# ChuhanZhou/News_Recommendation_Model

Measured on AMD Instinct MI355X. Metric: train impressions/sec, higher is better.
Workload: dtype f32

## Files before the change

### include/nrm_hotpath.h

```cpp
#ifndef NRM_HOTPATH_H
#define NRM_HOTPATH_H

#ifdef __cplusplus
extern "C" {
#endif

#define NRM_ABI_VERSION 7
#define NRM_OK 0
#define NRM_EINVAL (-1)
#define NRM_ELAUNCH (-2)

typedef void* nrm_stream_t;

int nrm_abi_version(void);
const char* nrm_last_error(void);
int nrm_build_flags(void);
const char* nrm_source_digest(void);
const char* nrm_build_info(void);


#define NRM_MMA_F32 0
#define NRM_MMA_BF16 1
#define NRM_MMA_BF16X3 2
long nrm_pwattn_packed_floats(int D);
int nrm_pwattn_pack_wp(const float* fc1_weight, int ld, int D, int mma, float* packed, nrm_stream_t stream);
int nrm_pwattn_fwd(const float* t, const float* h, const float* u, const float* v, const float* packed_wp,
                   const float* w2, const float* b2, float* z, float* s,
                   int B, int T, int H, int D, int mma, nrm_stream_t stream);

#define NRM_DZ_F32 0
#define NRM_DZ_HL4 1
int nrm_pwattn_bwd_dz(float* z_inout, const float* ds, const float* w2, float* dw2, float* db2, float* du, float* dv,
                      int B, int T, int H, int D, int dz_format, nrm_stream_t stream);
int nrm_pwattn_bwd_nsplit(int B, int T, int H, int D, int mma);
int nrm_pwattn_bwd_contract(const float* dz, const float* t, const float* h, const float* wp, int ldwp,
                            float* dt, float* dh, float* ws,
                            int B, int T, int H, int D, int passes, int mma, int dz_format, nrm_stream_t stream);
int nrm_pwattn_bwd_form(int T, int H, int D, int pass, int mma, int dz_format);
int nrm_pwattn_bwd_rw_supported(int D, int mma);
long nrm_pwattn_bwd_rw_packed_floats(int D, int mma);
int nrm_pwattn_bwd_rw_pack(const float* fc1_weight, int ld, int D, int mma, float* packed, nrm_stream_t stream);
int nrm_pwattn_bwd_rw_dtdh(const float* dz_hl4, const float* t, const float* h, const float* packed, float* dt, float* dh,
                           int B, int T, int H, int D, int mma, nrm_stream_t stream);

int nrm_pwattn_bwd_dp_supported(int D, int H);
long nrm_pwattn_bwd_dp_packed_floats(int D, int H);
int nrm_pwattn_bwd_dp_pack(const float* fc1_weight, int ld, int D, int H, float* packed, nrm_stream_t stream);
int nrm_pwattn_bwd_dp_dtdh(const float* dz, const float* t, const float* h, const float* packed, float* dt, float* dh,
                           int B, int T, int H, int D, nrm_stream_t stream);

#define NRM_EPI_BIAS 0
#define NRM_EPI_GELU 1
#define NRM_EPI_DGELU 2
#define NRM_EPI_MUL 3
long nrm_gemm_packed_floats(int nrows, int ncols, int mma);
int nrm_gemm_nt_bf16_supported(int M, int K, int mma);
int nrm_gemm_pack(const float* src, long row_stride, long col_stride, int nrows, int ncols, float* packed,
                  nrm_stream_t stream);
typedef struct {
    const float* src; const float* src2; float sign2;
    long row_stride, col_stride; int nrows, ncols;
    float* packed;
    int mma;
} nrm_pack_desc;
int nrm_gemm_pack_multi(const nrm_pack_desc* descs, int n, nrm_stream_t stream);
int nrm_gemm_nt(const float* x, int ldx, int M, const float* packed, int N, int K, const float* bias,
                float* y, int ldy, float* z, int ldz, const float* m, int ldm, int epilogue, int mma, nrm_stream_t stream);
int nrm_gemm_tn_nsplit(int ncols_i, int ncols_j, int R, int mma);
int nrm_gemm_tn(const float* A, int lda, int ncols_i, const float* B, int ldb, int ncols_j, int R,
                float* ws, int ldws, float* colsum, float* zero_out, long zero_n, int mma, nrm_stream_t stream);

int nrm_slab_reduce(const float* ws, int nsplit, int nj, int ldws, int ni, float* out, long out_istride, long out_jstride,
                    float* out2, long out2_istride, long out2_jstride, float sign2,
                    const float* vec, float* vec_out, nrm_stream_t stream);
typedef struct nrm_slab_desc {
    const float* ws; int nsplit, nj, ldws, ni;
    float* out; long out_istride, out_jstride;
    float* out2; long out2_istride, out2_jstride; float sign2;
    const float* vec; float* vec_out;
} nrm_slab_desc;
int nrm_slab_reduce_multi(const nrm_slab_desc* descs, int n, nrm_stream_t stream);

int nrm_head_fold(const float* w_o1, const float* b_o1, const float* w_m2, const float* b_m2, int P, int Q, int R,
                  float* packed_fwd, float* packed_bwd, float* bias, nrm_stream_t stream);
int nrm_head_fold_bwd(const float* dwp, int ldp, const float* dbp, const float* w_o1, const float* w_m2, const float* b_m2,
                      int P, int Q, int R, float* dw_o1, float* dw_m2, float* db_o1, float* db_m2, nrm_stream_t stream);

int nrm_colreduce(int mode, const float* x, const float* dy, const float* mean, const float* rstd,
                  float* s0, float* s1, int R, int N, int ld, nrm_stream_t stream);
int nrm_bn_finalize(int stage, const float* s, float* out, float* running, int R, int N, float momentum, float eps,
                    nrm_stream_t stream);
int nrm_mul_bwd(const float* dy, int lddy, const float* g, int ldg, const float* e, int lde, float* dg, float* de, int ldo,
                int R, int N, nrm_stream_t stream);
int nrm_bn_apply(const float* x, const float* mean, const float* rstd, const float* gamma, const float* beta,
                 float* y, int R, int N, int ld, nrm_stream_t stream);
int nrm_bn_backward(const float* x, const float* dy, const float* mean, const float* rstd, const float* gamma,
                    const float* s0, const float* s1, const float* add, float* dx, int R, int N, int ld, int training,
                    nrm_stream_t stream);
int nrm_concat_cols(const float* const* srcs, const long* lds, const int* widths, int n, float* out, int ldo, long R,
                    nrm_stream_t stream);

int nrm_pool_bmm(const float* W, long wsb, long wsi, long wsj, const float* X, int ldx, float* out,
                 int B, int I, int J, int D, int accumulate, nrm_stream_t stream);
int nrm_pool_rowdot(const float* g, int ldg, const float* h, float* ds, int B, int T, int H, int D, float* zero_out, int zero_n,
                    nrm_stream_t stream);

int nrm_small_linear_relu_fwd(const void* x, int x_is_f64, const float* weight, const float* bias, float* y, long R, int K, int N, int ldy,
                              nrm_stream_t stream);
int nrm_small_linear_relu_bwd(const void* x, int x_is_f64, const float* weight, const float* bias, const float* dy, int lddy, long R,
                              int K, int N, float* dwb, nrm_stream_t stream);

int nrm_loss_fwd_bwd(const float* out, int out_stride, const void* label, int label_is_f64, const long* user_id, const float* delta,
                     long n_delta, float alpha, int B, int T, float* loss_sum, float* dout, int dout_stride, float* ddelta, int* err,
                     nrm_stream_t stream);

int nrm_adam_step(float* p, float* g, float* m, float* v, long n, float lr, float beta1, float beta2, float eps,
                  float weight_decay, int step, int zero_grad, nrm_stream_t stream);
int nrm_gather_flat(const float* const* srcs, const long* offsets, const long* counts, int n, float* flat, long flat_n,
                    nrm_stream_t stream);
int nrm_adam_step_dev(float* p, float* g, float* m, float* v, long n, float lr, float beta1, float beta2, float eps,
                      float weight_decay, float* state, int zero_grad, nrm_stream_t stream);

int nrm_frontend_fwd(const void* x, int x_is_f64, int nrows, int xcols, int P, int n_sub, int behaviour,
                     const float* cat_tab, int n_cat, int e0, const float* sen_w, const float* sen_b, int e1,
                     const float* type_tab, int n_type, int e2,
                     const float* year_tab, const float* month_tab, const float* day_tab, const float* hour_tab,
                     int n_year, int n_month, int n_day, int n_hour, int e3,
                     float* lab, int ldlab, float* ti, int ldti, int* err, nrm_stream_t stream);
int nrm_frontend_bwd(const void* x, int x_is_f64, int nrows, int xcols, int P, int n_sub, int behaviour,
                     const float* dlab, int lddl, const float* sen_w, const float* sen_b,
                     int n_cat, int e0, int e1, int n_type, int e2, int n_year, int n_month, int n_day, int n_hour, int e3,
                     float* d_cat_tab, float* d_sen_w, float* d_sen_b, float* d_type_tab,
                     float* d_year_tab, float* d_month_tab, float* d_day_tab, float* d_hour_tab, nrm_stream_t stream);

long nrm_frontend_cat_ws_ints(int n_cat, long nrows_total, int n_sub);
int nrm_frontend_cat_grad(const void* x0, int nrows0, int xcols0, const float* dlab0, int lddl0,
                          const void* x1, int nrows1, int xcols1, const float* dlab1, int lddl1, int x_is_f64,
                          int P, int n_sub, int n_cat, int e0, float* d_cat_tab, int* ws, nrm_stream_t stream);

int nrm_row_auc(const float* score, const float* label, const int* len, int B, int T, float* auc, int* top1,
                nrm_stream_t stream);

int nrm_ensemble_rank_max_candidates(void);
int nrm_ensemble_rank(const float* const* logits, const long* row_stride, const long* col_stride, int M, const int* empty,
                      const float* label, int B, int T, float* score, int* rank, int* live, float* metrics, nrm_stream_t stream);

int nrm_compact_gather(const void* x_target, int target_cols, int target_is_f64, const void* x_global, int global_cols, int global_is_f64,
                       const int* cand_off, const int* pad_mult, int B, int T, int trim, int N,
                       void* xt_compact, void* xg_compact, int* flag, nrm_stream_t stream);
int nrm_pwattn_fwd_ragged(const float* t, const float* h, const float* u, const float* v, const float* packed_wp,
                          const float* w2, const float* b2, float* s, const int* cand_imp, const int* cand_off,
                          int B, int N, int max_count, int H, int D, int mma, nrm_stream_t stream);
int nrm_pool_bmm_ragged(const float* s, const float* h, float* out, const int* cand_off, int B, int N, int max_count, int H, int D,
                        nrm_stream_t stream);
int nrm_ensemble_rank_ragged(const float* const* logits, const long* col_stride, int M, const int* cand_off, const int* pad_mult, int N,
                             const float* label, int B, int T, float* score, int* rank, int* live, float* metrics, nrm_stream_t stream);

int nrm_history_len(const void* x_history, int cols, int is_f64, int B, int H, int* hist_len, nrm_stream_t stream);
int nrm_history_gather(const void* x_history, int cols, int is_f64, const int* hist_off, int B, int H, int R, int k_max, void* xh_compact,
                       nrm_stream_t stream);
int nrm_history_tiles(const int* cand_imp, const int* cand_off, const int* hist_off, const int* tile_pre, int B, int N, int R, int Mt,
                      void* tile_tab, nrm_stream_t stream);
int nrm_pwattn_fwd_hragged(const float* t, const float* h, const float* u, const float* v, const float* packed_wp,
                           const float* w2, const float* b2, float* s, const int* cand_imp, const int* cand_off, const int* hist_off,
                           const int* tile_pre, const void* tile_tab, int B, int N, int max_count, int R, int Mt, int k_max, int D, int mma,
                           nrm_stream_t stream);
int nrm_pool_bmm_hragged(const float* s, const float* h, float* out, const int* cand_off, const int* hist_off, const int* hist_mult,
                         const int* tile_pre, int B, int N, int max_count, int R, int Mt, int k_max, int D, nrm_stream_t stream);

#ifdef __cplusplus
}
#endif
#endif
```

### news_recommendation_model_amd/csrc/capi.hip

```cpp
#include <stdarg.h>
#include <stdint.h>
#include <stdio.h>
#include <stdlib.h>
#include <vector>

#include "../../include/nrm_hotpath.h"
#include "pwattn.hpp"
#include "gemm.hpp"
#include "head.hpp"
#include "pool_loss.hpp"
#include "frontend.hpp"
#include "scoring.hpp"
#include "compact.hpp"

static thread_local char g_err[512] = "";

static int fail(int code, const char* fmt, ...) {
    va_list ap;
    va_start(ap, fmt);
    vsnprintf(g_err, sizeof(g_err), fmt, ap);
    va_end(ap);
    return code;
}
static int check_hip(hipError_t e, const char* what) {
// ... 402 lines not shown
    return check_hip(nrm::head_fold_launch(p, (hipStream_t)stream), "head_fold");
}

int nrm_head_fold_bwd(const float* dwp, int ldp, const float* dbp, const float* w_o1, const float* w_m2, const float* b_m2,
                      int P, int Q, int R, float* dw_o1, float* dw_m2, float* db_o1, float* db_m2, nrm_stream_t stream) {
    if (!dwp || !dbp || !w_o1 || !w_m2) return fail(NRM_EINVAL, "nrm_head_fold_bwd: null pointer");
    if (P <= 0 || Q <= 0 || R <= 0 || ldp % 4 || ldp < R || !al16(dwp))
        return fail(NRM_EINVAL, "nrm_head_fold_bwd: P=%d Q=%d R=%d ldp=%d (ldp a multiple of 4 covering R, 16-byte aligned rows)", P, Q, R, ldp);
    nrm::HeadSplitParams p = {};
    p.dwp = dwp; p.ldp = ldp; p.dbp = dbp; p.wo = w_o1; p.wm = w_m2; p.bm = b_m2; p.dwo = dw_o1; p.dwm = dw_m2; p.dbo = db_o1; p.dbm = db_m2;
    p.P = P; p.Q = Q; p.R = R;
    return check_hip(nrm::head_fold_bwd_launch(p, (hipStream_t)stream), "head_fold_bwd");
}

static int check_bn(const char* fn, int R, int N, int ld) {
    if (R < 0 || N <= 0 || N % 4 || ld % 4 || ld < N) return fail(NRM_EINVAL, "%s: R=%d N=%d ld=%d (N, ld multiples of 4)", fn, R, N, ld);
    return NRM_OK;
}

int nrm_colreduce(int mode, const float* x, const float* dy, const float* mean, const float* rstd,
                  float* s0, float* s1, int R, int N, int ld, nrm_stream_t stream) {
    if (int rc = check_bn("nrm_colreduce", R, N, ld)) return rc;
    if (!x || !s0 || (mode >= 1 && !mean) || (mode == 2 && (!dy || !rstd || !s1)) || mode < 0 || mode > 2)
        return fail(NRM_EINVAL, "nrm_colreduce: bad argument for mode %d", mode);
    return check_hip(nrm::colred_launch(mode, x, dy, mean, rstd, s0, s1, R, N, ld, (hipStream_t)stream), "colreduce");
}

int nrm_bn_finalize(int stage, const float* s, float* out, float* running, int R, int N, float momentum, float eps,
                    nrm_stream_t stream) {
    if (!s || !out) return fail(NRM_EINVAL, "nrm_bn_finalize: null pointer");
    if ((stage != 0 && stage != 1) || R <= 0 || N <= 0) return fail(NRM_EINVAL, "nrm_bn_finalize: stage=%d R=%d N=%d", stage, R, N);
    return check_hip(nrm::bn_finalize_launch(stage, s, out, running, R, N, momentum, eps, (hipStream_t)stream), "bn_finalize");
}

int nrm_mul_bwd(const float* dy, int lddy, const float* g, int ldg, const float* e, int lde, float* dg, float* de, int ldo,
                int R, int N, nrm_stream_t stream) {
    if (!dy || !g || !e || !dg || !de) return fail(NRM_EINVAL, "nrm_mul_bwd: null pointer");
    if (R < 0 || N <= 0 || N % 4 || lddy % 4 || ldg % 4 || lde % 4 || ldo % 4 || lddy < N || ldg < N || lde < N || ldo < N ||
        !al16(dy) || !al16(g) || !al16(e) || !al16(dg) || !al16(de))
        return fail(NRM_EINVAL, "nrm_mul_bwd: R=%d N=%d (N and leading dimensions multiples of 4, 16-byte aligned rows)", R, N);
    return check_hip(nrm::mul_bwd_launch(dy, g, e, dg, de, R, N, lddy, ldg, lde, ldo, (hipStream_t)stream), "mul_bwd");
}

int nrm_bn_apply(const float* x, const float* mean, const float* rstd, const float* gamma, const float* beta,
                 float* y, int R, int N, int ld, nrm_stream_t stream) {
    if (int rc = check_bn("nrm_bn_apply", R, N, ld)) return rc;
    if (!x || !mean || !rstd || !gamma || !beta || !y) return fail(NRM_EINVAL, "nrm_bn_apply: null pointer");
    return check_hip(nrm::bn_apply_launch(x, mean, rstd, gamma, beta, y, R, N, ld, (hipStream_t)stream), "bn_apply");
}

int nrm_bn_backward(const float* x, const float* dy, const float* mean, const float* rstd, const float* gamma,
                    const float* s0, const float* s1, const float* add, float* dx, int R, int N, int ld, int training,
                    nrm_stream_t stream) {
    if (int rc = check_bn("nrm_bn_backward", R, N, ld)) return rc;
    if (!dy || !rstd || !gamma || !dx || (training && (!x || !mean || !s0 || !s1)))
        return fail(NRM_EINVAL, "nrm_bn_backward: null pointer");
    return check_hip(nrm::bn_bwd_launch(x, dy, mean, rstd, gamma, s0, s1, add, dx, R, N, ld, training, (hipStream_t)stream), "bn_backward");
}


int nrm_concat_cols(const float* const* srcs, const long* lds, const int* widths, int n, float* out, int ldo, long R,
                    nrm_stream_t stream) {
    if (!srcs || !lds || !widths || !out) return fail(NRM_EINVAL, "nrm_concat_cols: null pointer");
    if (n < 1 || n > nrm::CONCAT_MAX || R < 0) return fail(NRM_EINVAL, "nrm_concat_cols: n=%d (1..%d) R=%ld", n, nrm::CONCAT_MAX, R);
    nrm::ConcatTable tab = {};
    int total = 0;
    for (int i = 0; i < n; ++i) {
        if (!srcs[i] || widths[i] <= 0 || lds[i] < widths[i]) return fail(NRM_EINVAL, "nrm_concat_cols: part %d (width %d, ld %ld)", i, widths[i], lds[i]);
        tab.src[i] = srcs[i]; tab.ld[i] = lds[i]; tab.start[i] = total;
        total += widths[i];
    }
    tab.n = n;
    if (ldo < total) return fail(NRM_EINVAL, "nrm_concat_cols: ldo=%d < %d columns", ldo, total);
    return check_hip(nrm::concat_cols_launch(tab, out, R, ldo, total, (hipStream_t)stream), "concat_cols");
}

int nrm_pool_bmm(const float* W, long wsb, long wsi, long wsj, const float* X, int ldx, float* out,
                 int B, int I, int J, int D, int accumulate, nrm_stream_t stream) {
    if (!W || !X || !out) return fail(NRM_EINVAL, "nrm_pool_bmm: null pointer");
    if (B < 0 || I <= 0 || J <= 0 || D <= 0 || D % 4 || B > 65535) return fail(NRM_EINVAL, "nrm_pool_bmm: B=%d I=%d J=%d D=%d", B, I, J, D);
    if (ldx < D || ldx % 4 || !al16(X) || (long)J * ldx * 4 >= (1L << 31))
        return fail(NRM_EINVAL, "nrm_pool_bmm: ldx=%d (>= D, a multiple of 4, X 16-byte aligned, J*ldx*4 < 2^31)", ldx);
    return check_hip(nrm::bmm_rows_launch(W, wsb, wsi, wsj, X, (long)J * ldx, ldx, out, (long)I * D, D, B, I, J, D, accumulate,
                                          (hipStream_t)stream), "pool_bmm");
}

int nrm_pool_bmm_ragged(const float* s, const float* h, float* out, const int* cand_off, int B, int N, int max_count, int H, int D,
                        nrm_stream_t stream) {
    if (!s || !h || !out || !cand_off) return fail(NRM_EINVAL, "nrm_pool_bmm_ragged: null pointer");
    if (B < 0 || N < 0 || max_count < 0 || max_count > N || H <= 0 || D <= 0 || D % 4 || B > 65535)
        return fail(NRM_EINVAL, "nrm_pool_bmm_ragged: B=%d N=%d max_count=%d H=%d D=%d", B, N, max_count, H, D);
    if (!al16(h) || !al16(out) || (long)H * D * 4 >= (1L << 31) || (long)N * H >= (1L << 31))
        return fail(NRM_EINVAL, "nrm_pool_bmm_ragged: h and out must be 16-byte aligned, H*D*4 and N*H below 2^31");
    return check_hip(nrm::bmm_rows_ragged_launch(s, H, h, (long)H * D, D, out, D, cand_off, B, N, max_count, H, D, (hipStream_t)stream), "pool_bmm_ragged");
}

int nrm_pool_rowdot(const float* g, int ldg, const float* h, float* ds, int B, int T, int H, int D, float* zero_out, int zero_n,
                    nrm_stream_t stream) {
    if (!g || !h || !ds) return fail(NRM_EINVAL, "nrm_pool_rowdot: null pointer");
    if (B < 0 || T <= 0 || H <= 0 || D <= 0 || D % 4 || D > 1024 || B > 65535) return fail(NRM_EINVAL, "nrm_pool_rowdot: B=%d T=%d H=%d D=%d", B, T, H, D);
    if (ldg < D || ldg % 4 || !al16(g) || (long)T * ldg * 4 >= (1L << 31))
        return fail(NRM_EINVAL, "nrm_pool_rowdot: ldg=%d (>= D, a multiple of 4, g 16-byte aligned, T*ldg*4 < 2^31)", ldg);
    if (zero_n < 0 || (zero_n > 0 && !zero_out)) return fail(NRM_EINVAL, "nrm_pool_rowdot: zero_n=%d without zero_out", zero_n);
    return check_hip(nrm::rowdot_launch(g, (long)T * ldg, ldg, h, (long)H * D, D, ds, B, T, H, D, zero_out, zero_n, (hipStream_t)stream), "pool_rowdot");
}

int nrm_small_linear_relu_fwd(const void* x, int x_is_f64, const float* weight, const float* bias, float* y, long R, int K, int N, int ldy,
                              nrm_stream_t stream) {
    if (!x || !weight || !y) return fail(NRM_EINVAL, "nrm_small_linear_relu_fwd: null pointer");
    if (R < 0 || K < 1 || K > 4 || N < 1 || N > 8 || ldy < N) return fail(NRM_EINVAL, "nrm_small_linear_relu_fwd: R=%ld K=%d N=%d ldy=%d (K <= 4, N <= 8)", R, K, N, ldy);
    return check_hip(nrm::small_linear_relu_fwd_launch(x, x_is_f64, weight, bias, y, R, K, N, ldy, (hipStream_t)stream), "small_linear_relu_fwd");
}

int nrm_small_linear_relu_bwd(const void* x, int x_is_f64, const float* weight, const float* bias, const float* dy, int lddy, long R,
                              int K, int N, float* dwb, nrm_stream_t stream) {
    if (!x || !weight || !dy || !dwb) return fail(NRM_EINVAL, "nrm_small_linear_relu_bwd: null pointer");
    if (R < 0 || K < 1 || K > 4 || N < 1 || N > 8 || lddy < N) return fail(NRM_EINVAL, "nrm_small_linear_relu_bwd: R=%ld K=%d N=%d lddy=%d (K <= 4, N <= 8)", R, K, N, lddy);
    return check_hip(nrm::small_linear_relu_bwd_launch(x, x_is_f64, weight, bias, dy, lddy, R, K, N, dwb, (hipStream_t)stream), "small_linear_relu_bwd");
}

int nrm_loss_fwd_bwd(const float* out, int out_stride, const void* label, int label_is_f64, const long* user_id, const float* delta,
                     long n_delta, float alpha, int B, int T, float* loss_sum, float* dout, int dout_stride, float* ddelta, int* err,
                     nrm_stream_t stream) {
    if (!out || !label || !user_id || !delta || !loss_sum || !dout || !ddelta || !err) return fail(NRM_EINVAL, "nrm_loss_fwd_bwd: null pointer");
    if (B < 0 || T <= 0 || n_delta < 1 || (long)B * T >= (1L << 29))
        return fail(NRM_EINVAL, "nrm_loss_fwd_bwd: B=%d T=%d n_delta=%ld (T >= 1, n_delta >= 1, B*T < 2^29)", B, T, n_delta);
    if (out_stride < 1 || dout_stride < 1 || (dout_stride == 4 && !al16(dout)))
        return fail(NRM_EINVAL, "nrm_loss_fwd_bwd: out_stride=%d dout_stride=%d (>= 1; dout 16-byte aligned for stride 4)", out_stride, dout_stride);
    return check_hip(nrm::loss_launch(out, out_stride, label, label_is_f64, user_id, delta, n_delta, alpha, B, T, loss_sum, dout, dout_stride,
                                      ddelta, err, (hipStream_t)stream), "loss");
}

int nrm_adam_step(float* p, float* g, float* m, float* v, long n, float lr, float beta1, float beta2, float eps,
                  float weight_decay, int step, int zero_grad, nrm_stream_t stream) {
    if (!p || !g || !m || !v) return fail(NRM_EINVAL, "nrm_adam_step: null pointer");
    if (n < 0 || n % 4 || step < 1 || !al16(p) || !al16(g) || !al16(m) || !al16(v))
        return fail(NRM_EINVAL, "nrm_adam_step: n=%ld step=%d (n %% 4 == 0, step >= 1, 16-byte aligned buffers)", n, step);
    return check_hip(nrm::adam_launch(p, g, m, v, n, lr, beta1, beta2, eps, weight_decay, step, zero_grad, (hipStream_t)stream), "adam");
}


int nrm_gather_flat(const float* const* srcs, const long* offsets, const long* counts, int n, float* flat, long flat_n,
                    nrm_stream_t stream) {
    if ((n > 0 && (!srcs || !offsets || !counts)) || !flat) return fail(NRM_EINVAL, "nrm_gather_flat: null pointer");
    if (n < 0) return fail(NRM_EINVAL, "nrm_gather_flat: n=%d", n);
    for (int lo = 0; lo < n; lo += nrm::GATHER_MAX) {
        const int m = n - lo < nrm::GATHER_MAX ? n - lo : nrm::GATHER_MAX;
        nrm::GatherTable tab;
        long mx = 0;
        for (int i = 0; i < m; ++i) {
            if (offsets[lo + i] < 0 || counts[lo + i] < 0 || offsets[lo + i] + counts[lo + i] > flat_n)
                return fail(NRM_EINVAL, "nrm_gather_flat: entry %d (offset %ld, count %ld) leaves the flat buffer of %ld floats",
                            lo + i, offsets[lo + i], counts[lo + i], flat_n);
            tab.src[i] = srcs[lo + i]; tab.off[i] = offsets[lo + i]; tab.cnt[i] = counts[lo + i];
            if (counts[lo + i] > mx) mx = counts[lo + i];
        }
        if (int rc = check_hip(nrm::gather_flat_launch(tab, m, mx, flat, (hipStream_t)stream), "gather_flat")) return rc;
    }
    return NRM_OK;
}

int nrm_adam_step_dev(float* p, float* g, float* m, float* v, long n, float lr, float beta1, float beta2, float eps,
                      float weight_decay, float* state, int zero_grad, nrm_stream_t stream) {
    if (!p || !g || !m || !v || !state) return fail(NRM_EINVAL, "nrm_adam_step_dev: null pointer");
    if (n < 0 || n % 4 || !al16(p) || !al16(g) || !al16(m) || !al16(v))
        return fail(NRM_EINVAL, "nrm_adam_step_dev: n=%ld (n %% 4 == 0, 16-byte aligned buffers)", n);
    return check_hip(nrm::adam_dev_launch(p, g, m, v, n, lr, beta1, beta2, eps, weight_decay, state, zero_grad, (hipStream_t)stream), "adam_dev");
}

int nrm_row_auc(const float* score, const float* label, const int* len, int B, int T, float* auc, int* top1,
                nrm_stream_t stream) {
    if (!score || !label || !auc || !top1) return fail(NRM_EINVAL, "nrm_row_auc: null pointer");
    if (B < 0 || T <= 0) return fail(NRM_EINVAL, "nrm_row_auc: B=%d T=%d", B, T);
    return check_hip(nrm::row_auc_launch(score, label, len, B, T, auc, top1, (hipStream_t)stream), "row_auc");
}

int nrm_ensemble_rank_max_candidates(void) { return nrm::ENSEMBLE_MAX_CANDIDATES; }

int nrm_ensemble_rank(const float* const* logits, const long* row_stride, const long* col_stride, int M, const int* empty,
                      const float* label, int B, int T, float* score, int* rank, int* live, float* metrics, nrm_stream_t stream) {
    if (!logits || !row_stride || !score || !rank || !live) return fail(NRM_EINVAL, "nrm_ensemble_rank: null pointer");
    if (M < 1 || M > nrm::ENSEMBLE_MAX_MODELS) return fail(NRM_EINVAL, "nrm_ensemble_rank: M=%d models (1 .. %d)", M, nrm::ENSEMBLE_MAX_MODELS);
    if (B < 0 || T <= 0) return fail(NRM_EINVAL, "nrm_ensemble_rank: B=%d T=%d", B, T);
    if (T > nrm::ENSEMBLE_MAX_CANDIDATES)
        return fail(NRM_EINVAL, "nrm_ensemble_rank: T=%d candidates exceed the cap of %d (nrm_ensemble_rank_max_candidates)", T, nrm::ENSEMBLE_MAX_CANDIDATES);
    if ((label == nullptr) != (metrics == nullptr)) return fail(NRM_EINVAL, "nrm_ensemble_rank: label and metrics must be given together or both be NULL");
    nrm::EnsembleLogits lg = {};
    for (int m = 0; m < M; ++m) {
        if (!logits[m]) return fail(NRM_EINVAL, "nrm_ensemble_rank: logits[%d] is a null pointer", m);
        const long cs = col_stride ? col_stride[m] : 1;
        if (row_stride[m] < 0 || cs < 1) return fail(NRM_EINVAL, "nrm_ensemble_rank: model %d has row stride %ld, column stride %ld (need >= 0, >= 1)", m, row_stride[m], cs);
        lg.ptr[m] = logits[m]; lg.row_stride[m] = row_stride[m]; lg.col_stride[m] = cs;
    }
    return check_hip(nrm::ensemble_rank_launch(lg, M, empty, label, B, T, score, rank, live, metrics, (hipStream_t)stream), "ensemble_rank");
}

int nrm_pool_bmm_hragged(const float* s, const float* h, float* out, const int* cand_off, const int* hist_off, const int* hist_mult,
                         const int* tile_pre, int B, int N, int max_count, int R, int Mt, int k_max, int D, nrm_stream_t stream) {
    if (!s || !h || !out || !cand_off || !hist_off || !hist_mult || !tile_pre) return fail(NRM_EINVAL, "nrm_pool_bmm_hragged: null pointer");
    if (B < 0 || N < 0 || max_count < 0 || max_count > N || R < 0 || Mt < 0 || k_max < 0 || k_max > R || D <= 0 || D % 4)
        return fail(NRM_EINVAL, "nrm_pool_bmm_hragged: B=%d N=%d max_count=%d R=%d Mt=%d k_max=%d D=%d", B, N, max_count, R, Mt, k_max, D);
    if (((uintptr_t)h | (uintptr_t)out) & 15 || (long)R * D * 4 >= (1L << 31) || 16L * Mt >= (1L << 31))
        return fail(NRM_EINVAL, "nrm_pool_bmm_hragged: h and out must be 16-byte aligned, R*D*4 and 16*Mt below 2^31");
    if (R == 0 || Mt == 0) return NRM_OK;
    return check_hip(nrm::bmm_rows_hragged_launch(s, h, D, out, D, cand_off, hist_off, hist_mult, tile_pre, B, N, max_count, R, Mt, k_max, D,
                                                  (hipStream_t)stream), "pool_bmm_hragged");
}

int nrm_history_len(const void* x_history, int cols, int is_f64, int B, int H, int* hist_len, nrm_stream_t stream) {
    if (B < 0 || H < 0 || cols <= 0) return fail(NRM_EINVAL, "nrm_history_len: B=%d H=%d cols=%d", B, H, cols);
    const long words = (long)cols * (is_f64 ? 2 : 1);
    if ((long)H * words >= (1L << 31)) return fail(NRM_EINVAL, "nrm_history_len: H*cols=%ld words of one impression exceed 2^31", (long)H * words);
    if ((B > 0 && !hist_len) || (B > 0 && H > 0 && !x_history)) return fail(NRM_EINVAL, "nrm_history_len: null pointer");
    if ((uintptr_t)x_history & 3) return fail(NRM_EINVAL, "nrm_history_len: x_history must be 4-byte aligned");
    return check_hip(nrm::history_len_launch((const unsigned*)x_history, B, H, (int)words, hist_len, (hipStream_t)stream), "history_len");
}

int nrm_history_gather(const void* x_history, int cols, int is_f64, const int* hist_off, int B, int H, int R, int k_max, void* xh_compact,
                       nrm_stream_t stream) {
    if (B < 0 || H < 0 || cols <= 0 || R < 0 || k_max < 0 || k_max > H || (long)R > (long)B * H)
        return fail(NRM_EINVAL, "nrm_history_gather: B=%d H=%d cols=%d R=%d k_max=%d (0 <= k_max <= H, R <= B*H)", B, H, cols, R, k_max);
    if ((long)cols * 2 >= (1L << 31)) return fail(NRM_EINVAL, "nrm_history_gather: cols=%d", cols);
    if (!hist_off || (R > 0 && (!x_history || !xh_compact))) return fail(NRM_EINVAL, "nrm_history_gather: null pointer");
    return check_hip(nrm::history_gather_launch((const unsigned*)x_history, (unsigned*)xh_compact, cols * (is_f64 ? 2 : 1), hist_off, B, H, R, k_max,
                                                (hipStream_t)stream), "history_gather");
}

int nrm_history_tiles(const int* cand_imp, const int* cand_off, const int* hist_off, const int* tile_pre, int B, int N, int R, int Mt,
                      void* tile_tab, nrm_stream_t stream) {
    if (B < 0 || N < 0 || R < 0 || Mt < 0) return fail(NRM_EINVAL, "nrm_history_tiles: B=%d N=%d R=%d Mt=%d", B, N, R, Mt);
    if (16L * Mt >= (1L << 31)) return fail(NRM_EINVAL, "nrm_history_tiles: 16*Mt=%ld exceeds 2^31 rows", 16L * Mt);
    if (!cand_imp || !cand_off || !hist_off || !tile_pre || (Mt > 0 && !tile_tab)) return fail(NRM_EINVAL, "nrm_history_tiles: null pointer");
    if ((uintptr_t)tile_tab & 15) return fail(NRM_EINVAL, "nrm_history_tiles: tile_tab must be 16-byte aligned");
    return check_hip(nrm::history_tiles_launch(cand_imp, cand_off, hist_off, tile_pre, B, N, R, Mt, (int4*)tile_tab, (hipStream_t)stream), "history_tiles");
}

int nrm_ensemble_rank_ragged(const float* const* logits, const long* col_stride, int M, const int* cand_off, const int* pad_mult, int N,
                             const float* label, int B, int T, float* score, int* rank, int* live, float* metrics, nrm_stream_t stream) {
    if (!logits || !cand_off || !pad_mult || !score || !rank || !live) return fail(NRM_EINVAL, "nrm_ensemble_rank_ragged: null pointer");
    if (M < 1 || M > nrm::ENSEMBLE_MAX_MODELS) return fail(NRM_EINVAL, "nrm_ensemble_rank_ragged: M=%d models (1 .. %d)", M, nrm::ENSEMBLE_MAX_MODELS);
    if (B < 0 || T <= 0 || N < 0) return fail(NRM_EINVAL, "nrm_ensemble_rank_ragged: B=%d T=%d N=%d", B, T, N);
    if (T > nrm::ENSEMBLE_MAX_CANDIDATES)
        return fail(NRM_EINVAL, "nrm_ensemble_rank_ragged: T=%d candidates exceed the cap of %d (nrm_ensemble_rank_max_candidates)", T, nrm::ENSEMBLE_MAX_CANDIDATES);
    if ((label == nullptr) != (metrics == nullptr)) return fail(NRM_EINVAL, "nrm_ensemble_rank_ragged: label and metrics must be given together or both be NULL");
    nrm::EnsembleLogits lg = {};
    for (int m = 0; m < M; ++m) {
        if (!logits[m] && N > 0) return fail(NRM_EINVAL, "nrm_ensemble_rank_ragged: logits[%d] is a null pointer", m);
        const long cs = col_stride ? col_stride[m] : 1;
        if (cs < 1) return fail(NRM_EINVAL, "nrm_ensemble_rank_ragged: model %d has entry stride %ld (need >= 1)", m, cs);
        lg.ptr[m] = logits[m]; lg.row_stride[m] = 0; lg.col_stride[m] = cs;
    }
    return check_hip(nrm::ensemble_rank_ragged_launch(lg, M, cand_off, pad_mult, N, label, B, T, score, rank, live, metrics, (hipStream_t)stream),
                     "ensemble_rank_ragged");
}

int nrm_compact_gather(const void* x_target, int target_cols, int target_is_f64, const void* x_global, int global_cols, int global_is_f64,
                       const int* cand_off, const int* pad_mult, int B, int T, int trim, int N,
                       void* xt_compact, void* xg_compact, int* flag, nrm_stream_t stream) {
    if (B < 0 || T <= 0 || trim < 0 || trim > T || N < 0 || target_cols <= 0 || global_cols <= 0)
        return fail(NRM_EINVAL, "nrm_compact_gather: B=%d T=%d trim=%d N=%d target_cols=%d global_cols=%d", B, T, trim, N, target_cols, global_cols);
    if ((long)N > (long)B * (T - trim)) return fail(NRM_EINVAL, "nrm_compact_gather: N=%d compact rows exceed the B*(T - trim)=%ld kept cells", N, (long)B * (T - trim));
    if (!cand_off || !pad_mult || !flag || !x_target || !x_global || (N > 0 && (!xt_compact || !xg_compact))) return fail(NRM_EINVAL, "nrm_compact_gather: null pointer");
    nrm::CompactGatherParams p;
    p.xt = (const unsigned*)x_target; p.xg = (const unsigned*)x_global; p.xt_c = (unsigned*)xt_compact; p.xg_c = (unsigned*)xg_compact;
    p.wt = target_cols * (target_is_f64 ? 2 : 1); p.wg = global_cols * (global_is_f64 ? 2 : 1);
    p.cand_off = cand_off; p.pad_mult = pad_mult; p.B = B; p.T = T; p.Tp = T - trim; p.N = N; p.flag = flag;
    return check_hip(nrm::compact_gather_launch(p, (hipStream_t)stream), "compact_gather");
}

static int check_fe(const char* fn, int nrows, int xcols, int P, int n_sub, int behaviour, int e0, int e1, int e2, int e3) {
    if (nrows < 0 || P <= 0 || n_sub < 0 || e0 <= 0 || e1 <= 0 || e2 <= 0 || e3 <= 0)
        return fail(NRM_EINVAL, "%s: bad dimension", fn);
    if (n_sub > 16) return fail(NRM_EINVAL, "%s: n_sub=%d (<= 16 sub-category slots)", fn, n_sub);
    const int need = 4 + P + 1 + n_sub + 3 + 1 + (behaviour ? 2 : 0);
    if (xcols < need) return fail(NRM_EINVAL, "%s: packed rows have %d columns, layout needs %d", fn, xcols, need);
    return NRM_OK;
}

int nrm_frontend_fwd(const void* x, int x_is_f64, int nrows, int xcols, int P, int n_sub, int behaviour,
                     const float* cat_tab, int n_cat, int e0, const float* sen_w, const float* sen_b, int e1,
                     const float* type_tab, int n_type, int e2,
                     const float* year_tab, const float* month_tab, const float* day_tab, const float* hour_tab,
                     int n_year, int n_month, int n_day, int n_hour, int e3,
                     float* lab, int ldlab, float* ti, int ldti, int* err, nrm_stream_t stream) {
    if (int rc = check_fe("nrm_frontend_fwd", nrows, xcols, P, n_sub, behaviour, e0, e1, e2, e3)) return rc;
    if (!x || !cat_tab || !sen_w || !sen_b || !type_tab || !year_tab || !month_tab || !day_tab || !hour_tab || !lab || !ti || !err)
        return fail(NRM_EINVAL, "nrm_frontend_fwd: null pointer");
    if (ldlab < e0 + e1 + e2 + e3 + (behaviour ? 2 : 0) || ldti < P) return fail(NRM_EINVAL, "nrm_frontend_fwd: ldlab=%d ldti=%d too small", ldlab, ldti);
    nrm::FrontendParams p = {};
    p.cat_tab = cat_tab; p.sen_w = sen_w; p.sen_b = sen_b; p.type_tab = type_tab;
    p.year_tab = year_tab; p.month_tab = month_tab; p.day_tab = day_tab; p.hour_tab = hour_tab;
    p.n_cat = n_cat; p.n_type = n_type; p.n_year = n_year; p.n_month = n_month; p.n_day = n_day; p.n_hour = n_hour;
    p.e0 = e0; p.e1 = e1; p.e2 = e2; p.e3 = e3; p.P = P; p.n_sub = n_sub; p.xcols = xcols; p.behaviour = behaviour;
    p.lab = lab; p.ldlab = ldlab; p.ti = ti; p.ldti = ldti; p.err = err;
    return check_hip(nrm::frontend_fwd_launch(p, x, x_is_f64, nrows, (hipStream_t)stream), "frontend_fwd");
}

int nrm_frontend_bwd(const void* x, int x_is_f64, int nrows, int xcols, int P, int n_sub, int behaviour,
                     const float* dlab, int lddl, const float* sen_w, const float* sen_b,
                     int n_cat, int e0, int e1, int n_type, int e2, int n_year, int n_month, int n_day, int n_hour, int e3,
                     float* d_cat_tab, float* d_sen_w, float* d_sen_b, float* d_type_tab,
                     float* d_year_tab, float* d_month_tab, float* d_day_tab, float* d_hour_tab, nrm_stream_t stream) {
    if (int rc = check_fe("nrm_frontend_bwd", nrows, xcols, P, n_sub, behaviour, e0, e1, e2, e3)) return rc;
    if (!x || !dlab || !sen_w || !sen_b || !d_sen_w || !d_sen_b || !d_type_tab || !d_year_tab || !d_month_tab || !d_day_tab || !d_hour_tab)
        return fail(NRM_EINVAL, "nrm_frontend_bwd: null pointer");
    if (lddl < e0 + e1 + e2 + e3) return fail(NRM_EINVAL, "nrm_frontend_bwd: lddl=%d too small", lddl);
    nrm::FrontendParams p = {};
    p.sen_w = sen_w; p.sen_b = sen_b;
    p.d_cat_tab = d_cat_tab; p.d_sen_w = d_sen_w; p.d_sen_b = d_sen_b; p.d_type_tab = d_type_tab;
    p.d_year_tab = d_year_tab; p.d_month_tab = d_month_tab; p.d_day_tab = d_day_tab; p.d_hour_tab = d_hour_tab;
    p.n_cat = n_cat; p.n_type = n_type; p.n_year = n_year; p.n_month = n_month; p.n_day = n_day; p.n_hour = n_hour;
    p.e0 = e0; p.e1 = e1; p.e2 = e2; p.e3 = e3; p.P = P; p.n_sub = n_sub; p.xcols = xcols; p.behaviour = behaviour;
    return check_hip(nrm::frontend_bwd_launch(p, x, x_is_f64, dlab, lddl, nrows, (hipStream_t)stream), "frontend_bwd");
}

long nrm_frontend_cat_ws_ints(int n_cat, long nrows_total, int n_sub) {
    if (n_cat <= 0 || nrows_total < 0 || n_sub < 0) return 0;
    return nrm::cat_grad_ws_ints(n_cat, nrows_total, n_sub);
}

int nrm_frontend_cat_grad(const void* x0, int nrows0, int xcols0, const float* dlab0, int lddl0,
                          const void* x1, int nrows1, int xcols1, const float* dlab1, int lddl1, int x_is_f64,
                          int P, int n_sub, int n_cat, int e0, float* d_cat_tab, int* ws, nrm_stream_t stream) {
    if (nrows0 < 0 || nrows1 < 0 || P <= 0 || n_sub < 1 || n_sub > 16 || n_cat <= 0 || e0 <= 0 || e0 > 512)
        return fail(NRM_EINVAL, "nrm_frontend_cat_grad: nrows=%d,%d P=%d n_sub=%d n_cat=%d e0=%d (1 <= n_sub <= 16, e0 <= 512)", nrows0, nrows1, P, n_sub, n_cat, e0);
    if ((nrows0 > 0 && (!x0 || !dlab0 || lddl0 < e0 || xcols0 < 4 + P + 1 + n_sub)) || (nrows1 > 0 && (!x1 || !dlab1 || lddl1 < e0 || xcols1 < 4 + P + 1 + n_sub)) || !d_cat_tab || !ws)
        return fail(NRM_EINVAL, "nrm_frontend_cat_grad: null pointer, lddl < e0 or packed rows too short");
    if (((long)nrows0 + nrows1) * (n_sub + 1) >= (1L << 31)) return fail(NRM_EINVAL, "nrm_frontend_cat_grad: more than 2^31 table references");
    return check_hip(nrm::cat_grad_launch(x0, nrows0, xcols0, dlab0, lddl0, x1, nrows1, xcols1, dlab1, lddl1, x_is_f64, P, n_sub, n_cat, e0,
                                          d_cat_tab, ws, (hipStream_t)stream), "frontend_cat_grad");
}

}
```

### news_recommendation_model_amd/csrc/frontend.hip

```cpp
#include <algorithm>
#include "common.hpp"
#include "frontend.hpp"

namespace nrm {

template <typename XT>
__device__ __forceinline__ int row_index(const XT* xr, int col, int limit, int* err) {
    const int i = (int)xr[col];
    if (i < 0 || i >= limit) { *err = 1; return i < 0 ? 0 : limit - 1; }
    return i;
}

constexpr int FE_MAXSUB = 16;
constexpr int FE_HDR = 6 + FE_MAXSUB;
struct RowHeaders {
    int* idx;
    float* sen;
};

template <typename XT>
__device__ __forceinline__ void stage_headers(const FrontendParams& p, const XT* __restrict__ x, int r_lo, int nr, const RowHeaders& hd,
                                              int nthreads) {
    const int P = p.P, NS = p.n_sub;
    const int c_cat = 4 + P, c_sub = c_cat + 1, c_sen = c_sub + NS, c_typ = c_sen + 3;
    const int items = 9 + NS;
    for (int i = threadIdx.x; i < nr * items; i += nthreads) {
        const int r = i / items, k = i - r * items;
        const XT* xr = x + (size_t)(r_lo + r) * p.xcols;
        if (k < 4) {
            const int lim = k == 0 ? p.n_year : k == 1 ? p.n_month : k == 2 ? p.n_day : p.n_hour;
            hd.idx[r * FE_HDR + k] = row_index(xr, k, lim, p.err);
        } else if (k == 4) {
            hd.idx[r * FE_HDR + 4] = row_index(xr, c_cat, p.n_cat, p.err);
        } else if (k == 5) {
            hd.idx[r * FE_HDR + 5] = row_index(xr, c_typ, p.n_type, p.err);
        } else if (k < 6 + NS) {
            hd.idx[r * FE_HDR + k] = row_index(xr, c_sub + (k - 6), p.n_cat, p.err);
        } else {
            hd.sen[r * 4 + (k - 6 - NS)] = (float)xr[c_sen + (k - 6 - NS)];
        }
    }
}

constexpr int FWD_ROWS = 8;
constexpr int FE_THREADS = 256;

template <typename XT>
__global__ __launch_bounds__(FE_THREADS) void frontend_fwd_kernel(const FrontendParams p, const XT* __restrict__ x, int nrows) {
    __shared__ int h_idx[FWD_ROWS * FE_HDR];
    __shared__ float h_sen[FWD_ROWS * 4];
    const int r_lo = blockIdx.x * FWD_ROWS, nr = min(FWD_ROWS, nrows - r_lo);
    const RowHeaders hd = {h_idx, h_sen};
    stage_headers(p, x, r_lo, nr, hd, FE_THREADS);
    __syncthreads();
    const int P = p.P, NS = p.n_sub;
    const int c_beh = 4 + P + 1 + NS + 3 + 1;
    const int e0 = p.e0, e1 = p.e1, e2 = p.e2, e3 = p.e3;
    const int width = e0 + e1 + e2 + e3 + (p.behaviour ? 2 : 0);
    const float inv_ns = 1.0f / (float)NS;
    float* lab = p.lab + (size_t)r_lo * p.ldlab;
    for (int i = threadIdx.x; i < nr * p.ldlab; i += FE_THREADS) {
        const int r = i / p.ldlab, c = i - r * p.ldlab;
        const int* hi = h_idx + r * FE_HDR;
        float v = 0.f;
        if (c < e0) {
            float sub = 0.f;
            for (int k = 0; k < NS; ++k) sub += p.cat_tab[(size_t)hi[6 + k] * e0 + c];
            v = p.cat_tab[(size_t)hi[4] * e0 + c] + sub * inv_ns;
        } else if (c < e0 + e1) {
            const int j = c - e0;
            const float pre = p.sen_b[j] + p.sen_w[j * 3] * h_sen[r * 4] + p.sen_w[j * 3 + 1] * h_sen[r * 4 + 1] + p.sen_w[j * 3 + 2] * h_sen[r * 4 + 2];
            v = fmaxf(pre, 0.f);
        } else if (c < e0 + e1 + e2) {
            v = p.type_tab[(size_t)hi[5] * e2 + (c - e0 - e1)];
        } else if (c < e0 + e1 + e2 + e3) {
            const int k = c - e0 - e1 - e2;
            v = p.year_tab[(size_t)hi[0] * e3 + k] + p.month_tab[(size_t)hi[1] * e3 + k] + p.day_tab[(size_t)hi[2] * e3 + k] + p.hour_tab[(size_t)hi[3] * e3 + k];
        } else if (c < width) {
            v = (float)x[(size_t)(r_lo + r) * p.xcols + c_beh + (c - (e0 + e1 + e2 + e3))];
        }
        lab[i] = v;
    }
    float* ti = p.ti + (size_t)r_lo * p.ldti;
    for (int i = threadIdx.x; i < nr * p.ldti; i += FE_THREADS) {
        const int r = i / p.ldti, c = i - r * p.ldti;
        ti[i] = c < P ? (float)x[(size_t)(r_lo + r) * p.xcols + 4 + c] : 0.f;
    }
}

constexpr int FE_ROWS = 32;
constexpr int FE_MAX_BLOCKS = 512;

template <typename XT>
__global__ __launch_bounds__(FE_THREADS) void frontend_bwd_kernel(const FrontendParams p, const XT* __restrict__ x,
                                                                 const float* __restrict__ dlab, int lddl, int nrows) {
    extern __shared__ float sm[];
    const int e0 = p.e0, e1 = p.e1, e2 = p.e2, e3 = p.e3;
    float* a_type = sm;
    float* a_year = a_type + p.n_type * e2;
    float* a_month = a_year + p.n_year * e3;
    float* a_day = a_month + p.n_month * e3;
    float* a_hour = a_day + p.n_day * e3;
    float* a_sen = a_hour + p.n_hour * e3;
    const int total = (int)(a_sen + e1 * 4 - sm);
    const RowHeaders hd = {reinterpret_cast<int*>(sm + total), sm + total + FE_ROWS * FE_HDR};
    for (int i = threadIdx.x; i < total; i += FE_THREADS) sm[i] = 0.f;
    FrontendParams pq = p;
    int dummy = 0;
    pq.err = &dummy;
    const int NS = p.n_sub;
    const float inv_ns = 1.0f / (float)NS;
    const int small = e1 + e2 + e3;
    const int ngroups = (nrows + FE_ROWS - 1) / FE_ROWS;
    for (int grp = blockIdx.x; grp < ngroups; grp += gridDim.x) {
        const int r_lo = grp * FE_ROWS, nr = min(FE_ROWS, nrows - r_lo);
        __syncthreads();
        stage_headers(pq, x, r_lo, nr, hd, FE_THREADS);
        __syncthreads();
        const float* g0 = dlab + (size_t)r_lo * lddl;
        for (int i = threadIdx.x; i < (p.d_cat_tab ? nr * e0 : 0); i += FE_THREADS) {
            const int r = i / e0, c = i - r * e0;
            const int* hi = hd.idx + r * FE_HDR;
            const float gv = g0[(size_t)r * lddl + c];
            atomicAdd(p.d_cat_tab + (size_t)hi[4] * e0 + c, gv);
            const float gs = gv * inv_ns;
            for (int k = 0; k < NS; ++k) atomicAdd(p.d_cat_tab + (size_t)hi[6 + k] * e0 + c, gs);
        }
        for (int i = threadIdx.x; i < nr * small; i += FE_THREADS) {
            const int r = i / small, cs = i - r * small;
            const float gv = g0[(size_t)r * lddl + e0 + cs];
            const int* hi = hd.idx + r * FE_HDR;
            if (cs < e1) {
                const float s0 = hd.sen[r * 4], s1 = hd.sen[r * 4 + 1], s2 = hd.sen[r * 4 + 2];
                const float pre = p.sen_b[cs] + p.sen_w[cs * 3] * s0 + p.sen_w[cs * 3 + 1] * s1 + p.sen_w[cs * 3 + 2] * s2;
                if (pre > 0.f && gv != 0.f) {
                    atomicAdd(a_sen + cs * 4 + 0, gv * s0);
                    atomicAdd(a_sen + cs * 4 + 1, gv * s1);
                    atomicAdd(a_sen + cs * 4 + 2, gv * s2);
                    atomicAdd(a_sen + cs * 4 + 3, gv);
                }
            } else if (cs < e1 + e2) {
                atomicAdd(a_type + hi[5] * e2 + (cs - e1), gv);
            } else {
                const int k = cs - e1 - e2;
                atomicAdd(a_year + hi[0] * e3 + k, gv);
                atomicAdd(a_month + hi[1] * e3 + k, gv);
                atomicAdd(a_day + hi[2] * e3 + k, gv);
                atomicAdd(a_hour + hi[3] * e3 + k, gv);
            }
        }
    }
    __syncthreads();
    for (int i = threadIdx.x; i < p.n_type * e2; i += FE_THREADS) if (a_type[i] != 0.f) atomicAdd(p.d_type_tab + i, a_type[i]);
    for (int i = threadIdx.x; i < p.n_year * e3; i += FE_THREADS) if (a_year[i] != 0.f) atomicAdd(p.d_year_tab + i, a_year[i]);
    for (int i = threadIdx.x; i < p.n_month * e3; i += FE_THREADS) if (a_month[i] != 0.f) atomicAdd(p.d_month_tab + i, a_month[i]);
    for (int i = threadIdx.x; i < p.n_day * e3; i += FE_THREADS) if (a_day[i] != 0.f) atomicAdd(p.d_day_tab + i, a_day[i]);
    for (int i = threadIdx.x; i < p.n_hour * e3; i += FE_THREADS) if (a_hour[i] != 0.f) atomicAdd(p.d_hour_tab + i, a_hour[i]);
    for (int i = threadIdx.x; i < e1 * 4; i += FE_THREADS) {
        const float v = a_sen[i];
        if (v != 0.f) {
            const int j = i >> 2, w = i & 3;
            if (w < 3) atomicAdd(p.d_sen_w + j * 3 + w, v); else atomicAdd(p.d_sen_b + j, v);
        }
    }
}

static size_t bwd_lds_bytes(const FrontendParams& p) {
    return sizeof(float) * ((size_t)p.n_type * p.e2 + (size_t)(p.n_year + p.n_month + p.n_day + p.n_hour) * p.e3 + (size_t)p.e1 * 4 +
                            (size_t)FE_ROWS * (FE_HDR + 4));
}

hipError_t frontend_fwd_launch(const FrontendParams& p, const void* x, int x_is_f64, int nrows, hipStream_t st) {
    if (nrows <= 0) return hipSuccess;
    if (p.n_sub > FE_MAXSUB) return hipErrorInvalidValue;
    const dim3 grid((nrows + FWD_ROWS - 1) / FWD_ROWS);
    if (x_is_f64) hipLaunchKernelGGL(frontend_fwd_kernel<double>, grid, dim3(FE_THREADS), 0, st, p, (const double*)x, nrows);
    else          hipLaunchKernelGGL(frontend_fwd_kernel<float>, grid, dim3(FE_THREADS), 0, st, p, (const float*)x, nrows);
    return hipGetLastError();
}

hipError_t frontend_bwd_launch(const FrontendParams& p, const void* x, int x_is_f64, const float* dlab, int lddl,
                               int nrows, hipStream_t st) {
    if (nrows <= 0) return hipSuccess;
    const size_t shm = bwd_lds_bytes(p);
    if (shm > 160 * 1024 || p.n_sub > FE_MAXSUB) return hipErrorInvalidValue;
    const dim3 grid(std::min((nrows + FE_ROWS - 1) / FE_ROWS, FE_MAX_BLOCKS));
    if (x_is_f64) {
        if (shm > 64 * 1024) { hipError_t e = hipFuncSetAttribute((const void*)frontend_bwd_kernel<double>, hipFuncAttributeMaxDynamicSharedMemorySize, (int)shm); if (e != hipSuccess) return e; }
        hipLaunchKernelGGL(frontend_bwd_kernel<double>, grid, dim3(FE_THREADS), shm, st, p, (const double*)x, dlab, lddl, nrows);
    } else {
        if (shm > 64 * 1024) { hipError_t e = hipFuncSetAttribute((const void*)frontend_bwd_kernel<float>, hipFuncAttributeMaxDynamicSharedMemorySize, (int)shm); if (e != hipSuccess) return e; }
        hipLaunchKernelGGL(frontend_bwd_kernel<float>, grid, dim3(FE_THREADS), shm, st, p, (const float*)x, dlab, lddl, nrows);
    }
    return hipGetLastError();
}

struct CatRefs {
    const void* x[2]; const float* dlab[2];
    int nrows[2], xcols[2], lddl[2];
    int c_cat, NS, n_cat, e0;
    long nref;
};

template <typename XT>
__global__ __launch_bounds__(256) void cat_count_kernel(const CatRefs p, int* __restrict__ count, int* __restrict__ cat_of) {
    const int S = p.NS + 1;
    for (long i = (long)blockIdx.x * 256 + threadIdx.x; i < p.nref; i += (long)gridDim.x * 256) {
        long r = i / S;
        const int j = (int)(i - r * S);
        const int set = r >= p.nrows[0];
        if (set) r -= p.nrows[0];
        const XT* xr = reinterpret_cast<const XT*>(p.x[set]) + (size_t)r * p.xcols[set];
        int c = (int)xr[p.c_cat + j];
        c = c < 0 ? 0 : (c >= p.n_cat ? p.n_cat - 1 : c);
        cat_of[i] = c;
        atomicAdd(count + c, 1);
    }
}

__global__ __launch_bounds__(1024) void cat_scan_kernel(const int* __restrict__ count, int* __restrict__ start, int n) {
    __shared__ int part[1024];
    const int per = (n + 1023) / 1024;
    const int lo = threadIdx.x * per, hi = min(n, lo + per);
    int s = 0;
    for (int i = lo; i < hi; ++i) s += count[i];
    part[threadIdx.x] = s;
    __syncthreads();
    for (int off = 1; off < 1024; off <<= 1) {
        const int v = threadIdx.x >= off ? part[threadIdx.x - off] : 0;
        __syncthreads();
        part[threadIdx.x] += v;
        __syncthreads();
    }
    int run = threadIdx.x ? part[threadIdx.x - 1] : 0;
    for (int i = lo; i < hi; ++i) { start[i] = run; run += count[i]; }
    if (threadIdx.x == 1023) start[n] = part[1023];
}

__global__ __launch_bounds__(256) void cat_fill_kernel(long nref, const int* __restrict__ cat_of, const int* __restrict__ start,
                                                       int* __restrict__ cursor, int* __restrict__ refs, int* __restrict__ refcat) {
    for (long i = (long)blockIdx.x * 256 + threadIdx.x; i < nref; i += (long)gridDim.x * 256) {
        const int c = cat_of[i];
        const int pos = start[c] + atomicAdd(cursor + c, 1);
        refs[pos] = (int)i;
        refcat[pos] = c;
    }
}

constexpr int CAT_COLS = 8;
__global__ __launch_bounds__(256) void cat_gather_kernel(const CatRefs p, const int* __restrict__ refs, const int* __restrict__ refcat,
                                                         float* __restrict__ d_cat) {
    const int lane = threadIdx.x & 63;
    const long chunk = (long)blockIdx.x * 4 + (threadIdx.x >> 6);
    const long base = chunk * 64;
    if (base >= p.nref) return;
    const int S = p.NS + 1;
    const float inv_ns = 1.0f / (float)p.NS;
    const int my_ref = base + lane < p.nref ? refs[base + lane] : -1;
    const int my_cat = base + lane < p.nref ? refcat[base + lane] : -1;
    const int n_here = (int)min((long)64, p.nref - base);
    float acc[CAT_COLS];
#pragma unroll
    for (int k = 0; k < CAT_COLS; ++k) acc[k] = 0.f;
    int cur = __builtin_amdgcn_readfirstlane(my_cat);
    auto flush = [&](int c) {
        float* row = d_cat + (size_t)c * p.e0;
#pragma unroll
        for (int k = 0; k < CAT_COLS; ++k) {
            if (64 * k + lane < p.e0) atomicAdd(row + 64 * k + lane, acc[k]);
            acc[k] = 0.f;
        }
    };
    for (int t0 = 0; t0 < n_here; t0 += 4) {
        float v[4][CAT_COLS];
        int cs[4];
        float ws[4];
#pragma unroll
        for (int u = 0; u < 4; ++u) {
            const int t = t0 + u;
            const int i = __builtin_amdgcn_readlane(my_ref, t & 63);
            cs[u] = t < n_here ? __builtin_amdgcn_readlane(my_cat, t & 63) : -1;
            long r = i / S;
            const int j = i - (int)r * S;
            ws[u] = j ? inv_ns : 1.0f;
            const int set = r >= p.nrows[0];
            if (set) r -= p.nrows[0];
            const float* g = p.dlab[set] + (size_t)r * p.lddl[set];
#pragma unroll
            for (int k = 0; k < CAT_COLS; ++k) v[u][k] = (t < n_here && 64 * k + lane < p.e0) ? g[64 * k + lane] : 0.f;
        }
#pragma unroll
        for (int u = 0; u < 4; ++u) {
            if (cs[u] < 0) break;
            if (cs[u] != cur) { flush(cur); cur = cs[u]; }
#pragma unroll
            for (int k = 0; k < CAT_COLS; ++k) acc[k] = fmaf(ws[u], v[u][k], acc[k]);
        }
    }
    flush(cur);
}

long cat_grad_ws_ints(int n_cat, long nrows_total, int n_sub) { return 3L * n_cat + 4 + 3L * nrows_total * (n_sub + 1); }

hipError_t cat_grad_launch(const void* x0, int nrows0, int xcols0, const float* dlab0, int lddl0,
                           const void* x1, int nrows1, int xcols1, const float* dlab1, int lddl1, int x_is_f64,
                           int P, int n_sub, int n_cat, int e0, float* d_cat, int* ws, hipStream_t st) {
    CatRefs p = {};
    p.x[0] = x0; p.x[1] = x1; p.dlab[0] = dlab0; p.dlab[1] = dlab1;
    p.nrows[0] = nrows0; p.nrows[1] = nrows1; p.xcols[0] = xcols0; p.xcols[1] = xcols1; p.lddl[0] = lddl0; p.lddl[1] = lddl1;
    p.c_cat = 4 + P; p.NS = n_sub; p.n_cat = n_cat; p.e0 = e0;
    p.nref = ((long)nrows0 + nrows1) * (n_sub + 1);
    if (p.nref <= 0) return hipSuccess;
    if (e0 > 64 * CAT_COLS || n_sub < 1 || p.nref >= (1L << 31)) return hipErrorInvalidValue;
    int* count = ws;
    int* cursor = ws + n_cat;
    int* start = ws + 2 * n_cat;
    int* cat_of = ws + 3 * n_cat + 4;
    int* refs = cat_of + p.nref;
    int* refcat = refs + p.nref;
    hipError_t e = hipMemsetAsync(count, 0, sizeof(int) * 2 * (size_t)n_cat, st);
    if (e != hipSuccess) return e;
    const unsigned blocks = (unsigned)std::min<long>((p.nref + 255) / 256, 2048);
    if (x_is_f64) hipLaunchKernelGGL(cat_count_kernel<double>, dim3(blocks), dim3(256), 0, st, p, count, cat_of);
    else          hipLaunchKernelGGL(cat_count_kernel<float>, dim3(blocks), dim3(256), 0, st, p, count, cat_of);
    hipLaunchKernelGGL(cat_scan_kernel, dim3(1), dim3(1024), 0, st, count, start, n_cat);
    hipLaunchKernelGGL(cat_fill_kernel, dim3(blocks), dim3(256), 0, st, p.nref, cat_of, start, cursor, refs, refcat);
    const long chunks = (p.nref + 63) / 64;
    hipLaunchKernelGGL(cat_gather_kernel, dim3((unsigned)((chunks + 3) / 4)), dim3(256), 0, st, p, refs, refcat, d_cat);
    return hipGetLastError();
}

}
```

### news_recommendation_model_amd/csrc/frontend.hpp

```cpp
#pragma once
#include <hip/hip_runtime.h>

namespace nrm {
struct FrontendParams {
    const float *cat_tab, *sen_w, *sen_b, *type_tab, *year_tab, *month_tab, *day_tab, *hour_tab;
    float *d_cat_tab, *d_sen_w, *d_sen_b, *d_type_tab, *d_year_tab, *d_month_tab, *d_day_tab, *d_hour_tab;
    int n_cat, n_type, n_year, n_month, n_day, n_hour;
    int e0, e1, e2, e3;
    int P, n_sub, xcols, behaviour;
    float* lab; int ldlab;
    float* ti; int ldti;
    int* err;
};
hipError_t frontend_fwd_launch(const FrontendParams& p, const void* x, int x_is_f64, int nrows, hipStream_t st);
hipError_t frontend_bwd_launch(const FrontendParams& p, const void* x, int x_is_f64, const float* dlab, int lddl,
                               int nrows, hipStream_t st);
long cat_grad_ws_ints(int n_cat, long nrows_total, int n_sub);
hipError_t cat_grad_launch(const void* x0, int nrows0, int xcols0, const float* dlab0, int lddl0,
                           const void* x1, int nrows1, int xcols1, const float* dlab1, int lddl1, int x_is_f64,
                           int P, int n_sub, int n_cat, int e0, float* d_cat, int* ws, hipStream_t st);
}
```

### news_recommendation_model_amd/native.py

```python
from __future__ import annotations

import ctypes
import os
import threading

_HERE = os.path.dirname(os.path.abspath(__file__))
LIB_PATH = os.environ.get("NRM_HOTPATH_LIB") or os.path.join(_HERE, "libnrm_hotpath.so")
ABI_VERSION = 7

_c_fp = ctypes.c_void_p
_c_i, _c_l = ctypes.c_int, ctypes.c_long

SIGNATURES = {
    "nrm_abi_version": (_c_i, []),
    "nrm_last_error": (ctypes.c_char_p, []),
    "nrm_build_flags": (_c_i, []),
    "nrm_source_digest": (ctypes.c_char_p, []),
    "nrm_build_info": (ctypes.c_char_p, []),
    "nrm_pwattn_packed_floats": (_c_l, [_c_i]),
    "nrm_pwattn_pack_wp": (_c_i, [_c_fp, _c_i, _c_i, _c_i, _c_fp, _c_fp]),
    "nrm_pwattn_fwd": (_c_i, [_c_fp] * 9 + [_c_i] * 5 + [_c_fp]),
    "nrm_pwattn_bwd_dz": (_c_i, [_c_fp] * 7 + [_c_i] * 5 + [_c_fp]),
    "nrm_pwattn_bwd_rw_supported": (_c_i, [_c_i, _c_i]),
    "nrm_pwattn_bwd_rw_packed_floats": (_c_l, [_c_i, _c_i]),
    "nrm_pwattn_bwd_rw_pack": (_c_i, [_c_fp, _c_i, _c_i, _c_i, _c_fp, _c_fp]),
    "nrm_pwattn_bwd_rw_dtdh": (_c_i, [_c_fp] * 6 + [_c_i] * 5 + [_c_fp]),
    "nrm_pwattn_bwd_dp_supported": (_c_i, [_c_i, _c_i]),
    "nrm_pwattn_bwd_dp_packed_floats": (_c_l, [_c_i, _c_i]),
    "nrm_pwattn_bwd_dp_pack": (_c_i, [_c_fp, _c_i, _c_i, _c_i, _c_fp, _c_fp]),
    "nrm_pwattn_bwd_dp_dtdh": (_c_i, [_c_fp] * 6 + [_c_i] * 4 + [_c_fp]),
    "nrm_pwattn_bwd_nsplit": (_c_i, [_c_i] * 5),
    "nrm_pwattn_bwd_contract": (_c_i, [_c_fp] * 4 + [_c_i] + [_c_fp] * 3 + [_c_i] * 7 + [_c_fp]),
    "nrm_pwattn_bwd_form": (_c_i, [_c_i] * 6),
    "nrm_gemm_packed_floats": (_c_l, [_c_i, _c_i, _c_i]),
    "nrm_gemm_nt_bf16_supported": (_c_i, [_c_i, _c_i, _c_i]),
    "nrm_gemm_pack": (_c_i, [_c_fp, _c_l, _c_l, _c_i, _c_i, _c_fp, _c_fp]),
    "nrm_gemm_nt": (_c_i, [_c_fp, _c_i, _c_i, _c_fp, _c_i, _c_i, _c_fp, _c_fp, _c_i, _c_fp, _c_i, _c_fp, _c_i, _c_i, _c_i, _c_fp]),
    "nrm_slab_reduce": (_c_i, [_c_fp, _c_i, _c_i, _c_i, _c_i, _c_fp, _c_l, _c_l, _c_fp, _c_l, _c_l, ctypes.c_float,
                               _c_fp, _c_fp, _c_fp]),
    "nrm_bn_finalize": (_c_i, [_c_i, _c_fp, _c_fp, _c_fp, _c_i, _c_i, ctypes.c_float, ctypes.c_float, _c_fp]),
    "nrm_mul_bwd": (_c_i, [_c_fp, _c_i, _c_fp, _c_i, _c_fp, _c_i, _c_fp, _c_fp, _c_i, _c_i, _c_i, _c_fp]),
    "nrm_gemm_tn_nsplit": (_c_i, [_c_i, _c_i, _c_i, _c_i]),
    "nrm_gemm_tn": (_c_i, [_c_fp, _c_i, _c_i, _c_fp, _c_i, _c_i, _c_i, _c_fp, _c_i, _c_fp, _c_fp, _c_l, _c_i, _c_fp]),
    "nrm_gemm_pack_multi": (_c_i, [_c_fp, _c_i, _c_fp]),
    "nrm_slab_reduce_multi": (_c_i, [_c_fp, _c_i, _c_fp]),
    "nrm_head_fold": (_c_i, [_c_fp] * 4 + [_c_i] * 3 + [_c_fp] * 4),
    "nrm_head_fold_bwd": (_c_i, [_c_fp, _c_i, _c_fp, _c_fp, _c_fp, _c_fp, _c_i, _c_i, _c_i] + [_c_fp] * 5),
    "nrm_colreduce": (_c_i, [_c_i] + [_c_fp] * 6 + [_c_i] * 3 + [_c_fp]),
    "nrm_bn_apply": (_c_i, [_c_fp] * 6 + [_c_i] * 3 + [_c_fp]),
    "nrm_bn_backward": (_c_i, [_c_fp] * 9 + [_c_i] * 4 + [_c_fp]),
    "nrm_concat_cols": (_c_i, [_c_fp, _c_fp, _c_fp, _c_i, _c_fp, _c_i, _c_l, _c_fp]),
    "nrm_pool_bmm": (_c_i, [_c_fp, _c_l, _c_l, _c_l, _c_fp, _c_i, _c_fp] + [_c_i] * 5 + [_c_fp]),
    "nrm_pool_rowdot": (_c_i, [_c_fp, _c_i, _c_fp, _c_fp] + [_c_i] * 4 + [_c_fp, _c_i, _c_fp]),
    "nrm_small_linear_relu_fwd": (_c_i, [_c_fp, _c_i, _c_fp, _c_fp, _c_fp, _c_l, _c_i, _c_i, _c_i, _c_fp]),
    "nrm_small_linear_relu_bwd": (_c_i, [_c_fp, _c_i, _c_fp, _c_fp, _c_fp, _c_i, _c_l, _c_i, _c_i, _c_fp, _c_fp]),
    "nrm_loss_fwd_bwd": (_c_i, [_c_fp, _c_i, _c_fp, _c_i, _c_fp, _c_fp, _c_l, ctypes.c_float, _c_i, _c_i, _c_fp, _c_fp, _c_i, _c_fp, _c_fp, _c_fp]),
    "nrm_adam_step": (_c_i, [_c_fp] * 4 + [_c_l] + [ctypes.c_float] * 5 + [_c_i, _c_i, _c_fp]),
    "nrm_adam_step_dev": (_c_i, [_c_fp] * 4 + [_c_l] + [ctypes.c_float] * 5 + [_c_fp, _c_i, _c_fp]),
    "nrm_gather_flat": (_c_i, [_c_fp, _c_fp, _c_fp, _c_i, _c_fp, _c_l, _c_fp]),
    "nrm_row_auc": (_c_i, [_c_fp] * 3 + [_c_i, _c_i] + [_c_fp] * 3),
    "nrm_ensemble_rank_max_candidates": (_c_i, []),
    "nrm_ensemble_rank": (_c_i, [_c_fp] * 3 + [_c_i, _c_fp, _c_fp, _c_i, _c_i] + [_c_fp] * 5),
    "nrm_compact_gather": (_c_i, [_c_fp, _c_i, _c_i, _c_fp, _c_i, _c_i, _c_fp, _c_fp, _c_i, _c_i, _c_i, _c_i, _c_fp, _c_fp, _c_fp, _c_fp]),
    "nrm_pwattn_fwd_ragged": (_c_i, [_c_fp] * 10 + [_c_i] * 6 + [_c_fp]),
    "nrm_pool_bmm_ragged": (_c_i, [_c_fp] * 4 + [_c_i] * 5 + [_c_fp]),
    "nrm_history_len": (_c_i, [_c_fp, _c_i, _c_i, _c_i, _c_i, _c_fp, _c_fp]),
    "nrm_history_gather": (_c_i, [_c_fp, _c_i, _c_i, _c_fp, _c_i, _c_i, _c_i, _c_i, _c_fp, _c_fp]),
    "nrm_history_tiles": (_c_i, [_c_fp] * 4 + [_c_i] * 4 + [_c_fp, _c_fp]),
    "nrm_pwattn_fwd_hragged": (_c_i, [_c_fp] * 13 + [_c_i] * 8 + [_c_fp]),
    "nrm_pool_bmm_hragged": (_c_i, [_c_fp] * 7 + [_c_i] * 7 + [_c_fp]),
    "nrm_ensemble_rank_ragged": (_c_i, [_c_fp, _c_fp, _c_i, _c_fp, _c_fp, _c_i, _c_fp, _c_i, _c_i] + [_c_fp] * 5),
    "nrm_frontend_fwd": (_c_i, [_c_fp, _c_i, _c_i, _c_i, _c_i, _c_i, _c_i,  _c_fp, _c_i, _c_i,  _c_fp, _c_fp, _c_i,
                                 _c_fp, _c_i, _c_i,  _c_fp, _c_fp, _c_fp, _c_fp,  _c_i, _c_i, _c_i, _c_i, _c_i,
                                 _c_fp, _c_i, _c_fp, _c_i, _c_fp, _c_fp]),
    "nrm_frontend_cat_ws_ints": (_c_l, [_c_i, _c_l, _c_i]),
    "nrm_frontend_cat_grad": (_c_i, [_c_fp, _c_i, _c_i, _c_fp, _c_i] * 2 + [_c_i] * 5 + [_c_fp, _c_fp, _c_fp]),
    "nrm_frontend_bwd": (_c_i, [_c_fp, _c_i, _c_i, _c_i, _c_i, _c_i, _c_i,  _c_fp, _c_i, _c_fp, _c_fp]
                         + [_c_i] * 10 + [_c_fp] * 8 + [_c_fp]),
}



class PackDesc(ctypes.Structure):
    _fields_ = [("src", ctypes.c_void_p), ("src2", ctypes.c_void_p), ("sign2", ctypes.c_float),
                ("row_stride", ctypes.c_long), ("col_stride", ctypes.c_long), ("nrows", ctypes.c_int), ("ncols", ctypes.c_int),
                ("packed", ctypes.c_void_p), ("mma", ctypes.c_int)]


class SlabDesc(ctypes.Structure):
    _fields_ = [("ws", ctypes.c_void_p), ("nsplit", ctypes.c_int), ("nj", ctypes.c_int), ("ldws", ctypes.c_int), ("ni", ctypes.c_int),
                ("out", ctypes.c_void_p), ("out_istride", ctypes.c_long), ("out_jstride", ctypes.c_long),
                ("out2", ctypes.c_void_p), ("out2_istride", ctypes.c_long), ("out2_jstride", ctypes.c_long), ("sign2", ctypes.c_float),
                ("vec", ctypes.c_void_p), ("vec_out", ctypes.c_void_p)]


_lib = None
_lock = threading.Lock()


def load():
    global _lib
    if _lib is not None:
        return _lib
    with _lock:
        if _lib is not None:
            return _lib
        if not os.path.exists(LIB_PATH):
            raise RuntimeError(
                f"{LIB_PATH} is missing: build it with `python -m news_recommendation_model_amd.build` "
                "(hipcc --offload-arch=gfx950). There is no CPU or PyTorch fallback for the hot path.")
        lib = ctypes.CDLL(LIB_PATH)
        for name, (res, args) in SIGNATURES.items():
            fn = getattr(lib, name)
            fn.restype, fn.argtypes = res, args
        if lib.nrm_abi_version() != ABI_VERSION:
            raise RuntimeError(f"ABI mismatch: library {lib.nrm_abi_version()} != binding {ABI_VERSION}; rebuild")
        flags = lib.nrm_build_flags()
        if flags and os.environ.get("NRM_ALLOW_DIAG_LIB") != "1":
            raise RuntimeError(
                f"{LIB_PATH} is a timing-diagnostic build (nrm_build_flags() = {flags:#x}: kernels with parts of their work "
                "removed, results are wrong by construction); set NRM_ALLOW_DIAG_LIB=1 to load it for timing experiments")
        if os.environ.get("NRM_ALLOW_STALE_LIB") != "1" and not os.environ.get("NRM_HOTPATH_LIB"):
            from . import build as _build
            if os.path.isdir(_build.CSRC):
                have, want = lib.nrm_source_digest().decode(), _build.sources_digest()
                if have != want:
                    raise RuntimeError(f"{LIB_PATH} was built from other kernel sources (library {have[:16]}..., sources {want[:16]}...): "
                                       "rebuild with `python -m news_recommendation_model_amd.build` (NRM_ALLOW_STALE_LIB=1 loads it anyway)")
        _lib = lib
    return _lib


def provenance():
    lib = load()
    return {"library_sources_sha256": lib.nrm_source_digest().decode(), "build_info": lib.nrm_build_info().decode()}


kernel_events = None
kernel_event_tags = None


def call(name, *args, tag=None):
    lib = load()
    if kernel_events is not None and (kernel_event_tags is None or (tag or name) in kernel_event_tags):
        import torch
        e0, e1 = torch.cuda.Event(enable_timing=True), torch.cuda.Event(enable_timing=True)
        e0.record()
        rc = getattr(lib, name)(*args)
        e1.record()
        kernel_events.append((tag or name, e0, e1))
    else:
        rc = getattr(lib, name)(*args)
    if rc != 0:
        raise RuntimeError(f"{name} failed ({rc}): {lib.nrm_last_error().decode()}")


def ptr(t):
    return ctypes.c_void_p(t.data_ptr())


def stream_ptr():
    import torch
    return ctypes.c_void_p(torch.cuda.current_stream().cuda_stream)
```

### news_recommendation_model_amd/ops.py

```python
from __future__ import annotations

import torch

from . import native

EPI_BIAS, EPI_GELU, EPI_DGELU, EPI_MUL = 0, 1, 2, 3
MMA_F32, MMA_BF16, MMA_BF16X3 = 0, 1, 2
DZ_F32, DZ_HL4 = 0, 1
_MMA_NAMES = {"f32": MMA_F32, "fp32": MMA_F32, "float32": MMA_F32, "bf16": MMA_BF16, "bfloat16": MMA_BF16, "bf16x3": MMA_BF16X3}
_default_mma = MMA_F32


def resolve_mma(mma):
    if mma is None:
        return _default_mma
    if isinstance(mma, str):
        if mma.lower() not in _MMA_NAMES:
            raise ValueError(f"attention arithmetic {mma!r}: expected 'f32', 'bf16' or 'bf16x3'")
        return _MMA_NAMES[mma.lower()]
    if int(mma) not in (MMA_F32, MMA_BF16, MMA_BF16X3):
        raise ValueError(f"attention arithmetic {mma!r}: expected NRM_MMA_F32 (0), NRM_MMA_BF16 (1) or NRM_MMA_BF16X3 (2)")
    return int(mma)


# ... 1291 lines not shown
    out = torch.empty(B, T, D, dtype=torch.float32, device=h.device)
    native.call("nrm_pool_bmm", native.ptr(s), T * H, H, 1, native.ptr(h), D, native.ptr(out), B, T, H, D, 0,
                native.stream_ptr())
    return out


weighted_pool_fwd = _op("weighted_pool_fwd", "(Tensor scores, Tensor history) -> Tensor", _pool_fwd_impl,
                        lambda s, h: s.new_empty((s.shape[0], s.shape[1], h.shape[2]), dtype=torch.float32))


def _pooled_grad_rows(g, B, T, D):
    g = g if g.dtype == torch.float32 else g.to(torch.float32)
    ld = g.stride(1) if T > 1 else (g.stride(0) if B > 1 else D)
    if (g.dim() == 3 and g.stride(2) == 1 and ld >= D and ld % 4 == 0 and (B == 1 or g.stride(0) == T * ld)
            and (T == 1 or g.stride(1) == ld) and g.data_ptr() % 16 == 0 and T * ld * 4 < (1 << 31)):
        return g, ld
    return g.contiguous(), D


def _pool_bwd_impl(g, s, h):
    _require_gpu(g, s, h)
    s, h = _f32c(s), _f32c(h)
    B, T, H = s.shape
    D = h.shape[2]
    g, ldg = _pooled_grad_rows(g, B, T, D)
    st = native.stream_ptr()
    ds = torch.empty(B, T, H, dtype=torch.float32, device=h.device)
    native.call("nrm_pool_rowdot", native.ptr(g), ldg, native.ptr(h), native.ptr(ds), B, T, H, D, None, 0, st)
    dh = torch.empty(B, H, D, dtype=torch.float32, device=h.device)
    native.call("nrm_pool_bmm", native.ptr(s), T * H, 1, H, native.ptr(g), ldg, native.ptr(dh), B, H, T, D, 0, st)
    return ds, dh


weighted_pool_bwd = _op("weighted_pool_bwd", "(Tensor g, Tensor scores, Tensor history) -> (Tensor, Tensor)", _pool_bwd_impl,
                        lambda g, s, h: (s.new_empty(tuple(s.shape), dtype=torch.float32), h.new_empty(tuple(h.shape), dtype=torch.float32)))


def _pool_setup(ctx, inputs, output):
    ctx.save_for_backward(*inputs)


def _pool_backward(ctx, g):
    s, h = ctx.saved_tensors
    return weighted_pool_bwd(g, s, h)


torch.library.register_autograd("nrm::weighted_pool_fwd", _pool_backward, setup_context=_pool_setup, lib=_LIB)


def weighted_pool(scores, history):
    D = history.shape[-1]
    if scores.numel() == 0:
        return _degenerate((scores.shape[0], scores.shape[1], D), scores, history)
    _require_gpu(scores, history)
    if D % 4 == 0:
        return weighted_pool_fwd(scores, history)
    return weighted_pool_fwd(scores, torch.nn.functional.pad(history.to(torch.float32), (0, _pad4(D) - D)))[..., :D]


def _attend_pool_fwd_impl(t, h, w1, b1, w2, b2, save_z, mma):
    s, z = _pwattn_fwd_impl(t, h, w1, b1, w2, b2, save_z, mma)
    return _pool_fwd_impl(s, h), s, z


def _attend_pool_fwd_fake(t, h, w1, b1, w2, b2, save_z, mma):
    s, z = _pwattn_fwd_fake(t, h, w1, b1, w2, b2, save_z, mma)
    return t.new_empty(tuple(t.shape), dtype=torch.float32), s, z


attend_pool_fwd = _op("attend_pool_fwd", "(Tensor t, Tensor h, Tensor fc1_weight, Tensor fc1_bias, Tensor fc2_weight, Tensor fc2_bias, "
                      "bool save_z, int mma) -> (Tensor, Tensor, Tensor)", _attend_pool_fwd_impl, _attend_pool_fwd_fake)


def _attend_pool_bwd_impl(g, t, h, w1, w2, s, z, mma, need_dt, need_dh):
    _require_gpu(g, t, h, w1, w2, s, z)
    B, T, D = t.shape
    H = h.shape[1]
    s, h = _f32c(s), _f32c(h)
    g, ldg = _pooled_grad_rows(g, B, T, D)
    st = native.stream_ptr()
    dev = h.device
    acc = torch.empty(D + 4, dtype=torch.float32, device=dev)
    ds = torch.empty(B, T, H, dtype=torch.float32, device=dev)
    native.call("nrm_pool_rowdot", native.ptr(g), ldg, native.ptr(h), native.ptr(ds), B, T, H, D, native.ptr(acc), D + 4, st)
    dt, dh, dw1, db1, dw2b2 = _attn_bwd_core(ds, t, h, w1, w2, z, mma, need_dt, need_dh, acc=acc)
    if need_dh:
        native.call("nrm_pool_bmm", native.ptr(s), T * H, 1, H, native.ptr(g), ldg, native.ptr(dh), B, H, T, D, 1, st)
    return dt, dh, dw1, db1, dw2b2


attend_pool_bwd = _op("attend_pool_bwd", "(Tensor g, Tensor t, Tensor h, Tensor fc1_weight, Tensor fc2_weight, Tensor s, Tensor(a!) z, "
                      "int mma, bool need_dt, bool need_dh) -> (Tensor, Tensor, Tensor, Tensor, Tensor)", _attend_pool_bwd_impl,
                      lambda g, t, h, w1, w2, s, z, mma, need_dt, need_dh: _pwattn_bwd_fake(s, t, h, w1, w2, z, mma, need_dt, need_dh))


def _attend_pool_setup(ctx, inputs, output):
    t, h, w1, b1, w2, b2, save_z, mma = inputs
    pooled, s, z = output
    ctx.set_materialize_grads(False)
    ctx.save_z = save_z
    ctx.mma = mma
    ctx.consumed = False
    ctx.w2_shape, ctx.b2_shape = tuple(w2.shape), tuple(b2.shape)
    ctx.mark_non_differentiable(s, z)
    if save_z:
        ctx.save_for_backward(t, h, w1, w2, s, z, b1)


def _attend_pool_backward(ctx, g, _ds, _dz):
    if g is None:
        return None, None, None, None, None, None, None, None
    if not ctx.save_z:
        raise RuntimeError("pointwise attention: the forward ran with save_z=False (no-grad / inference call); there "
                           "is nothing to differentiate through")
    t, h, w1, w2, s, z, b1 = ctx.saved_tensors
    need = ctx.needs_input_grad
    dt, dh, dw1, db1, dw2b2 = attend_pool_bwd(g, t, h, w1, w2, s, _consume_z(ctx, z, t, h, w1, b1, w2), ctx.mma, bool(need[0]), bool(need[1]))
    D = t.shape[2]
    return ((dt if need[0] else None), (dh if need[1] else None), dw1, db1, dw2b2[:D].reshape(ctx.w2_shape),
            dw2b2[D:D + 1].reshape(ctx.b2_shape), None, None)


torch.library.register_autograd("nrm::attend_pool_fwd", _attend_pool_backward, setup_context=_attend_pool_setup, lib=_LIB)


def attend_and_pool(target, history, fc1_weight, fc1_bias, fc2_weight, fc2_bias, mma=None):
    D = target.shape[-1]
    if D % 4 or target.dim() != 3 or target.shape[0] * target.shape[1] * history.shape[1] == 0:
        return weighted_pool(pointwise_attention_scores(target, history, fc1_weight, fc1_bias, fc2_weight, fc2_bias, mma=mma), history)
    args = (target, history, fc1_weight, fc1_bias, fc2_weight, fc2_bias)
    _require_gpu(*args)
    save_z = torch.is_grad_enabled() and any(a.requires_grad for a in args)
    return attend_pool_fwd(*args, save_z, resolve_mma(mma))[0]


_index_error_flag = {}


BRANCH_STREAMS_MAX_ELEMS = 1 << 62
_branch_streams = {}


def branch_stream(like):
    key = like.device.index if like.device.index is not None else torch.cuda.current_device()
    st = _branch_streams.get(key)
    if st is None:
        st = _branch_streams[key] = torch.cuda.Stream(device=like.device)
    return st


def index_error_flag(device):
    device = torch.device(device)
    if device.index is None:
        device = torch.device(device.type, torch.cuda.current_device())
    key = str(device)
    if key not in _index_error_flag:
        _index_error_flag[key] = torch.zeros(1, dtype=torch.int32).pin_memory()
    return _index_error_flag[key]


def check_index_errors(device="cuda"):
    device = torch.device(device)
    flag = index_error_flag(device)
    torch.cuda.synchronize(device if device.index is not None else None)
    if int(flag[0]):
        flag.zero_()
        raise IndexError("index out of range (a category / type / time table index of a packed feature row, or a user id "
                         "outside delta)")


def _loss_impl(out, delta, label, user_id, alpha):
    _require_gpu(out, delta, label, user_id)
    B, T = out.shape
    d = _f32c(delta)
    so = out.stride(1) if T > 1 else (out.stride(0) if B > 1 else 1)
    if not (out.dtype == torch.float32 and so >= 1 and (T == 1 or out.stride(1) == so) and (B == 1 or out.stride(0) == T * so)):
        out, so = _f32c(out), 1
    y = label if (label.dtype in (torch.float32, torch.float64) and label.is_contiguous()) else _f32c(label)
    uid = user_id.to(torch.int64).contiguous()
    loss = torch.zeros((), dtype=torch.float32, device=out.device)
    ddelta = torch.zeros_like(d)
    dbuf = torch.empty(B * T, 4, dtype=torch.float32, device=out.device)
    native.call("nrm_loss_fwd_bwd", native.ptr(out), so, native.ptr(y), 1 if y.dtype == torch.float64 else 0, native.ptr(uid),
                native.ptr(d), d.numel(), float(alpha), B, T, native.ptr(loss), native.ptr(dbuf), 4, native.ptr(ddelta),
                native.ptr(index_error_flag(out.device)), native.stream_ptr())
    return loss, dbuf[:, 0].view(B, T), ddelta


softmax_bce_loss_op = _op("softmax_bce_loss", "(Tensor out, Tensor delta, Tensor label, Tensor user_id, float alpha) -> "
                          "(Tensor, Tensor, Tensor)", _loss_impl,
                          lambda out, delta, label, user_id, alpha: (out.new_empty((), dtype=torch.float32),
                                                                     out.new_empty((out.shape[0] * out.shape[1], 4), dtype=torch.float32)[:, 0]
                                                                     .view(out.shape[0], out.shape[1]),
                                                                     delta.new_empty(tuple(delta.shape), dtype=torch.float32)))


def _loss_setup(ctx, inputs, output):
    ctx.set_materialize_grads(False)
    ctx.save_for_backward(output[1], output[2])


_unit_grads = {}


def unit_grad(like):
    key = like.device.index if like.device.index is not None else torch.cuda.current_device()
    u = _unit_grads.get(key)
    if u is None:
        if torch.cuda.is_current_stream_capturing():
            return None
        u = _unit_grads[key] = torch.ones((), dtype=torch.float32, device=like.device)
    return u


def _loss_backward(ctx, gl, _a, _b):
    if gl is None:
        return None, None, None, None, None
    dout, ddelta = ctx.saved_tensors
    u = _unit_grads.get(dout.device.index)
    try:
        unit = u is not None and gl.dim() == 0 and gl.data_ptr() == u.data_ptr()
    except RuntimeError:
        unit = False
    if unit:
        return dout, ddelta.clone(), None, None, None
    return dout * gl, ddelta * gl, None, None, None


torch.library.register_autograd("nrm::softmax_bce_loss", _loss_backward, setup_context=_loss_setup, lib=_LIB)


def softmax_bce_loss(out, delta, label, user_id, alpha):
    if out.numel() == 0:
        return _degenerate((), out, delta) + float("nan")
    _require_gpu(out, delta, label, user_id)
    return softmax_bce_loss_op(out, delta, label, user_id, float(alpha))[0]


def _frontend_dims(cat_tab, sen_w, type_tab, year_tab, month_tab, day_tab, hour_tab):
    return (cat_tab.shape[0], cat_tab.shape[1], sen_w.shape[0], type_tab.shape[0], type_tab.shape[1], year_tab.shape[0],
            month_tab.shape[0], day_tab.shape[0], hour_tab.shape[0], year_tab.shape[1])


def _frontend_fwd_impl(x, behaviour, n_sub, P, cat_tab, sen_w, sen_b, type_tab, year_tab, month_tab, day_tab, hour_tab):
    _require_gpu(x, cat_tab)
    if x.dtype not in (torch.float32, torch.float64):
        x = x.to(torch.float32)
    x = x.contiguous()
    R, xcols = x.shape
    tabs = [_f32c(t) for t in (cat_tab, sen_w, sen_b, type_tab, year_tab, month_tab, day_tab, hour_tab)]
    cat_tab, sen_w, sen_b, type_tab, year_tab, month_tab, day_tab, hour_tab = tabs
    dims = _frontend_dims(cat_tab, sen_w, type_tab, year_tab, month_tab, day_tab, hour_tab)
    n_cat, e0, e1, n_type, e2, n_year, n_month, n_day, n_hour, e3 = dims
    width = e0 + e1 + e2 + e3 + (2 if behaviour else 0)
    ldlab, ldti = _pad4(width), _pad4(P)
    lab = torch.empty(R, ldlab, dtype=torch.float32, device=x.device)
    ti = torch.empty(R, ldti, dtype=torch.float32, device=x.device)
    native.call("nrm_frontend_fwd", native.ptr(x), 1 if x.dtype == torch.float64 else 0, R, xcols, P, n_sub,
                1 if behaviour else 0, native.ptr(cat_tab), n_cat, e0, native.ptr(sen_w), native.ptr(sen_b), e1,
                native.ptr(type_tab), n_type, e2, native.ptr(year_tab), native.ptr(month_tab), native.ptr(day_tab),
                native.ptr(hour_tab), n_year, n_month, n_day, n_hour, e3,
                native.ptr(lab), ldlab, native.ptr(ti), ldti, native.ptr(index_error_flag(x.device)),
                native.stream_ptr())
    return lab[:, :width], ti[:, :P]


def _frontend_fwd_fake(x, behaviour, n_sub, P, cat_tab, sen_w, sen_b, type_tab, year_tab, month_tab, day_tab, hour_tab):
    width = cat_tab.shape[1] + sen_w.shape[0] + type_tab.shape[1] + year_tab.shape[1] + (2 if behaviour else 0)
    return _padded_empty(x, x.shape[0], width), _padded_empty(x, x.shape[0], P)


_FRONT_TABLES = "Tensor cat_tab, Tensor sen_w, Tensor sen_b, Tensor type_tab, Tensor year_tab, Tensor month_tab, Tensor day_tab, Tensor hour_tab"
frontend_fwd = _op("frontend_fwd", f"(Tensor x, bool behaviour, int n_sub, int P, {_FRONT_TABLES}) -> (Tensor, Tensor)",
                   _frontend_fwd_impl, _frontend_fwd_fake)


def _frontend_bwd_impl(dlab, x, behaviour, n_sub, P, cat_tab, sen_w, sen_b, type_tab, year_tab, month_tab, day_tab, hour_tab):
    tabs = (cat_tab, sen_w, sen_b, type_tab, year_tab, month_tab, day_tab, hour_tab)
    return _frontend_bwd_sets([(dlab, x, behaviour)], n_sub, P, tabs)


FE_SORT_MIN_ATOMICS = 50_000_000


def _frontend_bwd_sets(sets, n_sub, P, tabs):
    cat_tab, sen_w, sen_b, type_tab, year_tab, month_tab, day_tab, hour_tab = tabs
    dev = sets[0][1].device
    sen_w, sen_b = _f32c(sen_w), _f32c(sen_b)
    dims = _frontend_dims(cat_tab, sen_w, type_tab, year_tab, month_tab, day_tab, hour_tab)
    n_cat, e0, e1, n_type, e2, n_year, n_month, n_day, n_hour, e3 = dims
    grads, arena = _frontend_grad_arena(tabs, dev)
    d_cat, d_sw, d_sb, d_type, d_year, d_month, d_day, d_hour = grads
    prepared = []
    for dlab, x, behaviour in sets:
        _require_gpu(dlab, x)
        if x.dtype not in (torch.float32, torch.float64):
            x = x.to(torch.float32)
        prepared.append((_rows(dlab), x.contiguous(), behaviour))
    refs = sum(x.shape[0] for _, x, _ in prepared) * (n_sub + 1)
    forced = _os.environ.get("NRM_FE_SORT")
    sort = (forced != "0" and (forced == "1" or refs * e0 >= FE_SORT_MIN_ATOMICS) and 1 <= n_sub <= 16 and e0 <= 512
            and len({x.dtype for _, x, _ in prepared}) == 1 and refs < (1 << 31))
    st = native.stream_ptr()
    for dlab, x, behaviour in prepared:
        native.call("nrm_frontend_bwd", native.ptr(x), 1 if x.dtype == torch.float64 else 0, x.shape[0], x.shape[1], P,
                    n_sub, 1 if behaviour else 0, native.ptr(dlab), dlab.stride(0), native.ptr(sen_w), native.ptr(sen_b),
                    n_cat, e0, e1, n_type, e2, n_year, n_month, n_day, n_hour, e3,
                    None if sort else native.ptr(d_cat), native.ptr(d_sw), native.ptr(d_sb), native.ptr(d_type),
                    native.ptr(d_year), native.ptr(d_month), native.ptr(d_day), native.ptr(d_hour), st)
    if sort:
        (dl0, x0, _), (dl1, x1, _) = prepared[0], (prepared[1] if len(prepared) > 1 else (None, None, None))
        rows = x0.shape[0] + (x1.shape[0] if x1 is not None else 0)
        ws = torch.empty(native.load().nrm_frontend_cat_ws_ints(n_cat, rows, n_sub), dtype=torch.int32, device=dev)
        native.call("nrm_frontend_cat_grad", native.ptr(x0), x0.shape[0], x0.shape[1], native.ptr(dl0), dl0.stride(0),
                    native.ptr(x1) if x1 is not None else None, x1.shape[0] if x1 is not None else 0,
                    x1.shape[1] if x1 is not None else 0, native.ptr(dl1) if x1 is not None else None,
                    dl1.stride(0) if x1 is not None else 0, 1 if x0.dtype == torch.float64 else 0, P, n_sub, n_cat, e0,
                    native.ptr(d_cat), native.ptr(ws), st)
    return arena


def _frontend_arena_floats(tabs):
    return sum(_pad4(int(t.numel())) for t in tabs)


def _frontend_bwd_fake(dlab, x, behaviour, n_sub, P, cat_tab, sen_w, sen_b, type_tab, year_tab, month_tab, day_tab, hour_tab):
    tabs = (cat_tab, sen_w, sen_b, type_tab, year_tab, month_tab, day_tab, hour_tab)
    return cat_tab.new_empty((_frontend_arena_floats(tabs),), dtype=torch.float32)


frontend_bwd = _op("frontend_bwd", f"(Tensor dlab, Tensor x, bool behaviour, int n_sub, int P, {_FRONT_TABLES}) -> Tensor",
                   _frontend_bwd_impl, _frontend_bwd_fake)


def _frontend_setup(ctx, inputs, output):
    ctx.set_materialize_grads(False)
    ctx.args = inputs[1:4]
    ctx.save_for_backward(inputs[0], *inputs[4:])


def _frontend_backward(ctx, dlab, _dti):
    if dlab is None:
        return (None,) * 12
    x, *tabs = ctx.saved_tensors
    arena = frontend_bwd(dlab, x, *ctx.args, *tabs)
    return (None, None, None, None) + _frontend_grad_arena(tabs, arena.device, arena)[0]


torch.library.register_autograd("nrm::frontend_fwd", _frontend_backward, setup_context=_frontend_setup, lib=_LIB)


def frontend(x, behaviour, n_sub, P, cat_tab, sen_w, sen_b, type_tab, year_tab, month_tab, day_tab, hour_tab):
    B, N = x.shape[0], x.shape[1]
    tabs = (cat_tab, sen_w, sen_b, type_tab, year_tab, month_tab, day_tab, hour_tab)
    if B * N == 0:
        width = cat_tab.shape[1] + sen_w.shape[0] + type_tab.shape[1] + year_tab.shape[1] + (2 if behaviour else 0)
        return _degenerate((B, N, width), x, *tabs), _degenerate((B, N, int(P)), x)
    _require_gpu(x, cat_tab)
    lab, ti = frontend_fwd(x.reshape(B * N, x.shape[2]), bool(behaviour), int(n_sub), int(P), *tabs)
    ti = ti.detach()
    return lab.reshape(B, N, -1) if lab.is_contiguous() else lab.unflatten(0, (B, N)), ti.unflatten(0, (B, N))


def _frontend_pair_fwd_impl(xh, xt, n_sub, P, cat_tab, sen_w, sen_b, type_tab, year_tab, month_tab, day_tab, hour_tab):
    tabs = (cat_tab, sen_w, sen_b, type_tab, year_tab, month_tab, day_tab, hour_tab)
    lab_h, ti_h = _frontend_fwd_impl(xh, True, n_sub, P, *tabs)
    lab_t, ti_t = _frontend_fwd_impl(xt, False, n_sub, P, *tabs)
    return lab_h, ti_h, lab_t, ti_t


def _frontend_pair_fwd_fake(xh, xt, n_sub, P, *tabs):
    return _frontend_fwd_fake(xh, True, n_sub, P, *tabs) + _frontend_fwd_fake(xt, False, n_sub, P, *tabs)


frontend_pair_fwd = _op("frontend_pair_fwd", f"(Tensor x_history, Tensor x_target, int n_sub, int P, {_FRONT_TABLES}) -> "
                        "(Tensor, Tensor, Tensor, Tensor)", _frontend_pair_fwd_impl, _frontend_pair_fwd_fake)


def _frontend_pair_bwd_impl(dlab_h, dlab_t, xh, xt, n_sub, P, cat_tab, sen_w, sen_b, type_tab, year_tab, month_tab, day_tab, hour_tab):
    tabs = (cat_tab, sen_w, sen_b, type_tab, year_tab, month_tab, day_tab, hour_tab)
    sets = [(dlab, x, beh) for dlab, x, beh in ((dlab_h, xh, True), (dlab_t, xt, False)) if dlab is not None]
    if not sets:
        return _frontend_grad_arena(tabs, xh.device)[1]
    return _frontend_bwd_sets(sets, n_sub, P, tabs)


def _frontend_grad_arena(tabs, dev, arena=None):
    cat_tab, sen_w, sen_b, type_tab, year_tab, month_tab, day_tab, hour_tab = tabs
    shapes = [tuple(cat_tab.shape), tuple(sen_w.shape), tuple(sen_b.shape), tuple(type_tab.shape), tuple(year_tab.shape),
              tuple(month_tab.shape), tuple(day_tab.shape), tuple(hour_tab.shape)]
    sizes = [_pad4(int(torch.Size(sh).numel())) for sh in shapes]
    if arena is None:
        arena = torch.zeros(sum(sizes), dtype=torch.float32, device=dev)
    grads, o = [], 0
    for sh, n in zip(shapes, sizes):
        grads.append(arena[o:o + int(torch.Size(sh).numel())].view(sh))
        o += n
    return tuple(grads), arena


frontend_pair_bwd = _op("frontend_pair_bwd", f"(Tensor? dlab_history, Tensor? dlab_target, Tensor x_history, Tensor x_target, int n_sub, int P, "
                        f"{_FRONT_TABLES}) -> Tensor", _frontend_pair_bwd_impl,
                        lambda dh, dt, xh, xt, n_sub, P, *tabs: tabs[0].new_empty((_frontend_arena_floats(tabs),), dtype=torch.float32))


def _frontend_pair_setup(ctx, inputs, output):
    ctx.set_materialize_grads(False)
    ctx.args = inputs[2:4]
    ctx.save_for_backward(inputs[0], inputs[1], *inputs[4:])


def _frontend_pair_backward(ctx, dlab_h, _dti_h, dlab_t, _dti_t):
    if dlab_h is None and dlab_t is None:
        return (None,) * 12
    xh, xt, *tabs = ctx.saved_tensors
    arena = frontend_pair_bwd(dlab_h, dlab_t, xh, xt, *ctx.args, *tabs)
    return (None, None, None, None) + _frontend_grad_arena(tabs, arena.device, arena)[0]


torch.library.register_autograd("nrm::frontend_pair_fwd", _frontend_pair_backward, setup_context=_frontend_pair_setup, lib=_LIB)


def frontend_pair(x_history, x_target, n_sub, P, cat_tab, sen_w, sen_b, type_tab, year_tab, month_tab, day_tab, hour_tab):
    tabs = (cat_tab, sen_w, sen_b, type_tab, year_tab, month_tab, day_tab, hour_tab)
    B, H, T = x_history.shape[0], x_history.shape[1], x_target.shape[1]
    if B * H == 0 or B * T == 0 or x_target.shape[0] != B:
        return frontend(x_history, True, n_sub, P, *tabs) + frontend(x_target, False, n_sub, P, *tabs)
    _require_gpu(x_history, x_target, cat_tab)
    lab_h, ti_h, lab_t, ti_t = frontend_pair_fwd(x_history.reshape(B * H, x_history.shape[2]), x_target.reshape(B * T, x_target.shape[2]),
                                                 int(n_sub), int(P), *tabs)
    shape = lambda a, n: a.reshape(B, n, -1) if a.is_contiguous() else a.unflatten(0, (B, n))
    return shape(lab_h, H), ti_h.detach().unflatten(0, (B, H)), shape(lab_t, T), ti_t.detach().unflatten(0, (B, T))


def _row_auc_impl(score, label, length):
    _require_gpu(score, label, length)
    s, y = _f32c(score), _f32c(label)
    B, T = s.shape
    auc = torch.empty(B, dtype=torch.float32, device=s.device)
    top1 = torch.empty(B, dtype=torch.int32, device=s.device)
    ln = length.to(torch.int32).contiguous() if length is not None else None
    native.call("nrm_row_auc", native.ptr(s), native.ptr(y), native.ptr(ln) if ln is not None else None, B, T,
                native.ptr(auc), native.ptr(top1), native.stream_ptr())
    return auc, top1


row_auc = _op("row_auc", "(Tensor score, Tensor label, Tensor? length) -> (Tensor, Tensor)", _row_auc_impl,
              lambda score, label, length: (score.new_empty((score.shape[0],), dtype=torch.float32),
                                            score.new_empty((score.shape[0],), dtype=torch.int32)))


def _ensemble_rank_impl(logits, empty, label):
    import ctypes
    logits = list(logits)
    _require_gpu(*logits, empty, label)
    if not logits or any(x.dim() != 2 or x.shape != logits[0].shape for x in logits):
        raise RuntimeError(f"ensemble_rank: needs 1 .. 8 logit matrices of one [B, T] shape, got {[tuple(x.shape) for x in logits]}")
    B, T = logits[0].shape
    xs = [x if (x.dtype == torch.float32 and (B <= 1 or x.stride(0) >= 0) and (T <= 1 or x.stride(1) >= 1)) else _f32c(x) for x in logits]
    M, dev = len(xs), xs[0].device
    score = torch.empty(B, T, dtype=torch.float32, device=dev)
    rank = torch.empty(B, T, dtype=torch.int32, device=dev)
    live = torch.empty(B, dtype=torch.int32, device=dev)
    metrics = torch.empty(B if label is not None else 0, 3, dtype=torch.float32, device=dev)
    if empty is not None and tuple(empty.shape) != (B,):
        raise RuntimeError(f"ensemble_rank: empty has shape {tuple(empty.shape)}, expected ({B},)")
    if label is not None and tuple(label.shape) != (B, T):
        raise RuntimeError(f"ensemble_rank: label has shape {tuple(label.shape)}, expected ({B}, {T})")
    em = empty.to(torch.int32).contiguous() if empty is not None else None
    y = _f32c(label) if label is not None else None
    ptrs = (ctypes.c_void_p * M)(*[x.data_ptr() for x in xs])
    rows = (ctypes.c_long * M)(*[x.stride(0) if B > 1 else 0 for x in xs])
    cols = (ctypes.c_long * M)(*[x.stride(1) if T > 1 else 1 for x in xs])
    native.call("nrm_ensemble_rank", ptrs, rows, cols, M, native.ptr(em) if em is not None else None,
                native.ptr(y) if y is not None else None, B, T, native.ptr(score), native.ptr(rank), native.ptr(live),
                native.ptr(metrics) if y is not None else None, native.stream_ptr())
    return score, rank, live, metrics


def _ensemble_rank_fake(logits, empty, label):
    x = logits[0]
    B, T = x.shape
    return (x.new_empty((B, T), dtype=torch.float32), x.new_empty((B, T), dtype=torch.int32), x.new_empty((B,), dtype=torch.int32),
            x.new_empty((B if label is not None else 0, 3), dtype=torch.float32))


ensemble_rank = _op("ensemble_rank", "(Tensor[] logits, Tensor? empty, Tensor? label) -> (Tensor score, Tensor rank, Tensor live, Tensor metrics)",
                    _ensemble_rank_impl, _ensemble_rank_fake)


_pad_error_flag = {}


def pad_error_flag(device):
    device = torch.device(device)
    if device.index is None:
        device = torch.device(device.type, torch.cuda.current_device())
    key = str(device)
    if key not in _pad_error_flag:
        _pad_error_flag[key] = torch.zeros(1, dtype=torch.int32).pin_memory()
    return _pad_error_flag[key]


def check_pad_errors(device="cuda"):
    device = torch.device(device)
    flag = pad_error_flag(device)
    torch.cuda.synchronize(device if device.index is not None else None)
    if int(flag[0]):
        flag.zero_()
        raise ValueError("compact scoring: a padded candidate row differs from the other padded rows of its impression (or the "
                         "plan does not match the batch): the padded logits are not all alike, score this data with the dense path")


def _tab(t):
    return t if (t.dtype == torch.int32 and t.is_contiguous()) else t.to(torch.int32).contiguous()


def _compact_gather_impl(x_target, x_global, cand_off, pad_mult, trim, N):
    _require_gpu(x_target, x_global, cand_off, pad_mult)
    fix = lambda x: (x if x.dtype in (torch.float32, torch.float64) else x.to(torch.float32)).contiguous()
    xt, xg = fix(x_target), fix(x_global)
    B, T = xt.shape[0], xt.shape[1]
    if xt.dim() != 3 or xg.dim() != 3 or tuple(xg.shape[:2]) != (B, T) or tuple(cand_off.shape) != (B + 1,) or tuple(pad_mult.shape) != (B,):
        raise RuntimeError(f"compact_gather: x_target {tuple(xt.shape)}, x_global {tuple(xg.shape)}, cand_off {tuple(cand_off.shape)}, "
                           f"pad_mult {tuple(pad_mult.shape)} do not agree")
    out_t = torch.empty(N, xt.shape[2], dtype=xt.dtype, device=xt.device)
    out_g = torch.empty(N, xg.shape[2], dtype=xg.dtype, device=xt.device)
    if B * T == 0:
        return out_t, out_g
    native.call("nrm_compact_gather", native.ptr(xt), xt.shape[2], 1 if xt.dtype == torch.float64 else 0,
                native.ptr(xg), xg.shape[2], 1 if xg.dtype == torch.float64 else 0, native.ptr(_tab(cand_off)), native.ptr(_tab(pad_mult)),
                B, T, int(trim), int(N), native.ptr(out_t), native.ptr(out_g), native.ptr(pad_error_flag(xt.device)), native.stream_ptr())
    return out_t, out_g


def _compact_gather_fake(x_target, x_global, cand_off, pad_mult, trim, N):
    f = lambda x: x.dtype if x.dtype in (torch.float32, torch.float64) else torch.float32
    return (x_target.new_empty((N, x_target.shape[2]), dtype=f(x_target)), x_global.new_empty((N, x_global.shape[2]), dtype=f(x_global)))


compact_gather = _op("compact_gather", "(Tensor x_target, Tensor x_global, Tensor cand_off, Tensor pad_mult, int trim, int N) -> (Tensor, Tensor)",
                     _compact_gather_impl, _compact_gather_fake)


def _attend_pool_ragged_fwd_impl(t, h, w1, b1, w2, b2, cand_imp, cand_off, max_count, mma):
    _require_gpu(t, h, w1, b1, w2, b2, cand_imp, cand_off)
    if mma != MMA_F32:
        raise RuntimeError("compact scoring: the ragged attention forward has fp32 arithmetic only; this attention is set to "
                           f"{ {MMA_BF16: 'bf16', MMA_BF16X3: 'bf16x3'}.get(mma, mma)} -- score with the dense path, or set the attention "
                           "arithmetic to 'f32'")
    N, D = t.shape
    B, H = h.shape[0], h.shape[1]
    if h.shape[2] != D or tuple(w1.shape) != (D, 4 * D) or D % 4 or tuple(cand_imp.shape) != (N,) or tuple(cand_off.shape) != (B + 1,):
        raise RuntimeError(f"ragged attention: target {tuple(t.shape)}, history {tuple(h.shape)}, fc1 {tuple(w1.shape)}, cand_imp "
                           f"{tuple(cand_imp.shape)}, cand_off {tuple(cand_off.shape)} do not agree (feature width must be a multiple of 4)")
    w1_arg = w1
    t, h, w1, b1 = _f32c(t), _f32c(h), _f32c(w1), _f32c(b1)
    w2v, b2 = _f32c(w2).reshape(-1), _f32c(b2).reshape(-1)
    s = torch.empty(N, H, dtype=torch.float32, device=t.device)
    pooled = torch.empty(N, D, dtype=torch.float32, device=t.device)
    if N == 0 or B * H == 0:
        return pooled.zero_(), s.zero_()
    cand_imp, cand_off = _tab(cand_imp), _tab(cand_off)
    own = w1 if w1 is w1_arg else None
    w_h, w_t, w_d = w1[:, :D], w1[:, D:2 * D], w1[:, 2 * D:3 * D]
    u, _ = _gemm_nt(h.reshape(B * H, D), w_h, 4 * D, 1, D, D, b1, EPI_BIAS, src2=w_d, sign2=-1.0, owner=own, mma=mma)
    v, _ = _gemm_nt(t, w_t, 4 * D, 1, D, D, None, EPI_BIAS, src2=w_d, sign2=1.0, owner=own, mma=mma)
    st = native.stream_ptr()
    packed = torch.empty(native.load().nrm_pwattn_packed_floats(D), dtype=torch.float32, device=t.device)
    native.call("nrm_pwattn_pack_wp", native.ptr(w1), 4 * D, D, mma, native.ptr(packed), st)
    _count_flops("contraction", 2.0 * N * H * D * D)
    native.call("nrm_pwattn_fwd_ragged", native.ptr(t), native.ptr(h), native.ptr(u), native.ptr(v), native.ptr(packed), native.ptr(w2v),
                native.ptr(b2), native.ptr(s), native.ptr(cand_imp), native.ptr(cand_off), B, N, int(max_count), H, D, mma, st,
                tag="pwattn_fwd_ragged")
    native.call("nrm_pool_bmm_ragged", native.ptr(s), native.ptr(h), native.ptr(pooled), native.ptr(cand_off), B, N, int(max_count), H, D, st)
    return pooled, s


attend_pool_ragged_fwd = _op("attend_pool_ragged_fwd", "(Tensor t, Tensor h, Tensor fc1_weight, Tensor fc1_bias, Tensor fc2_weight, Tensor fc2_bias, "
                             "Tensor cand_imp, Tensor cand_off, int max_count, int mma) -> (Tensor, Tensor)", _attend_pool_ragged_fwd_impl,
                             lambda t, h, w1, b1, w2, b2, ci, co, mc, mma: (t.new_empty(tuple(t.shape), dtype=torch.float32),
                                                                            t.new_empty((t.shape[0], h.shape[1]), dtype=torch.float32)))


def attend_pool_ragged(target, history, fc1_weight, fc1_bias, fc2_weight, fc2_bias, cand_imp, cand_off, max_count, mma=None):
    D = target.shape[-1]
    args = (target, history, fc1_weight, fc1_bias, fc2_weight, fc2_bias)
    _require_gpu(*args)
    if D % 4:
        P = _pad4(D) - D
        pad = torch.nn.functional.pad
        blocks = [pad(fc1_weight[:, i * D:(i + 1) * D], (0, P, 0, P)) for i in range(4)]
        args = (pad(target.to(torch.float32), (0, P)), pad(history.to(torch.float32), (0, P)), torch.cat(blocks, dim=1),
                pad(fc1_bias, (0, P)), pad(fc2_weight.reshape(1, D), (0, P)), fc2_bias)
    with torch.no_grad():
        return attend_pool_ragged_fwd(*args, cand_imp, cand_off, int(max_count), resolve_mma(mma))[0][:, :D]


def _history_len_impl(x_history):
    _require_gpu(x_history)
    x = (x_history if x_history.dtype in (torch.float32, torch.float64) else x_history.to(torch.float32)).contiguous()
    if x.dim() != 3:
        raise RuntimeError(f"history_len: x_history {tuple(x.shape)} is not [B, H, cols]")
    B, H, cols = x.shape
    out = torch.zeros(B, dtype=torch.int32, device=x.device)
    if B * H * cols:
        native.call("nrm_history_len", native.ptr(x), cols, 1 if x.dtype == torch.float64 else 0, B, H, native.ptr(out), native.stream_ptr())
    return out


history_len = _op("history_len", "(Tensor x_history) -> Tensor", _history_len_impl,
                  lambda x: x.new_empty((x.shape[0],), dtype=torch.int32))


def _history_gather_impl(x_history, hist_off, R, k_max):
# ... 146 lines not shown
```

Before: 35330.

## Add tiled matrix-core reduction kernel for small frontend table gradients

```diff
diff --git a/include/nrm_hotpath.h b/include/nrm_hotpath.h
--- a/include/nrm_hotpath.h
+++ b/include/nrm_hotpath.h
@@ -133,6 +133,14 @@
                      float* d_cat_tab, float* d_sen_w, float* d_sen_b, float* d_type_tab,
                      float* d_year_tab, float* d_month_tab, float* d_day_tab, float* d_hour_tab, nrm_stream_t stream);
 
+long nrm_frontend_tables_ws_floats(long nrows_total, int n_sub, int e1, int n_type, int e2, int n_year, int n_month, int n_day, int n_hour, int e3);
+int nrm_frontend_bwd_tables(const void* x0, int nrows0, int xcols0, int behaviour0, const float* dlab0, int lddl0,
+                            const void* x1, int nrows1, int xcols1, int behaviour1, const float* dlab1, int lddl1, int x_is_f64,
+                            int P, int n_sub, const float* sen_w, const float* sen_b,
+                            int e0, int e1, int n_type, int e2, int n_year, int n_month, int n_day, int n_hour, int e3,
+                            float* d_sen_w, float* d_sen_b, float* d_type_tab,
+                            float* d_year_tab, float* d_month_tab, float* d_day_tab, float* d_hour_tab, float* ws, nrm_stream_t stream);
+
 long nrm_frontend_cat_ws_ints(int n_cat, long nrows_total, int n_sub);
 int nrm_frontend_cat_grad(const void* x0, int nrows0, int xcols0, const float* dlab0, int lddl0,
                           const void* x1, int nrows1, int xcols1, const float* dlab1, int lddl1, int x_is_f64,
diff --git a/news_recommendation_model_amd/csrc/capi.hip b/news_recommendation_model_amd/csrc/capi.hip
--- a/news_recommendation_model_amd/csrc/capi.hip
+++ b/news_recommendation_model_amd/csrc/capi.hip
@@ -728,7 +728,8 @@
                      float* d_cat_tab, float* d_sen_w, float* d_sen_b, float* d_type_tab,
                      float* d_year_tab, float* d_month_tab, float* d_day_tab, float* d_hour_tab, nrm_stream_t stream) {
     if (int rc = check_fe("nrm_frontend_bwd", nrows, xcols, P, n_sub, behaviour, e0, e1, e2, e3)) return rc;
-    if (!x || !dlab || !sen_w || !sen_b || !d_sen_w || !d_sen_b || !d_type_tab || !d_year_tab || !d_month_tab || !d_day_tab || !d_hour_tab)
+    const int n_small = !!d_sen_w + !!d_sen_b + !!d_type_tab + !!d_year_tab + !!d_month_tab + !!d_day_tab + !!d_hour_tab;
+    if (!x || !dlab || !sen_w || !sen_b || (n_small != 7 && (n_small != 0 || !d_cat_tab)))
         return fail(NRM_EINVAL, "nrm_frontend_bwd: null pointer");
     if (lddl < e0 + e1 + e2 + e3) return fail(NRM_EINVAL, "nrm_frontend_bwd: lddl=%d too small", lddl);
     nrm::FrontendParams p = {};
@@ -738,6 +739,42 @@
     p.n_cat = n_cat; p.n_type = n_type; p.n_year = n_year; p.n_month = n_month; p.n_day = n_day; p.n_hour = n_hour;
     p.e0 = e0; p.e1 = e1; p.e2 = e2; p.e3 = e3; p.P = P; p.n_sub = n_sub; p.xcols = xcols; p.behaviour = behaviour;
     return check_hip(nrm::frontend_bwd_launch(p, x, x_is_f64, dlab, lddl, nrows, (hipStream_t)stream), "frontend_bwd");
+}
+
+static nrm::FrontendParams tab_dims(int n_sub, int e1, int n_type, int e2, int n_year, int n_month, int n_day, int n_hour, int e3) {
+    nrm::FrontendParams p = {};
+    p.n_type = n_type; p.n_year = n_year; p.n_month = n_month; p.n_day = n_day; p.n_hour = n_hour;
+    p.e1 = e1; p.e2 = e2; p.e3 = e3; p.n_sub = n_sub;
+    return p;
+}
+
+long nrm_frontend_tables_ws_floats(long nrows_total, int n_sub, int e1, int n_type, int e2, int n_year, int n_month, int n_day, int n_hour, int e3) {
+    if (nrows_total <= 0 || n_sub < 0) return 0;
+    return nrm::tab_grad_ws_floats(tab_dims(n_sub, e1, n_type, e2, n_year, n_month, n_day, n_hour, e3), nrows_total);
+}
+
+int nrm_frontend_bwd_tables(const void* x0, int nrows0, int xcols0, int behaviour0, const float* dlab0, int lddl0,
+                            const void* x1, int nrows1, int xcols1, int behaviour1, const float* dlab1, int lddl1, int x_is_f64,
+                            int P, int n_sub, const float* sen_w, const float* sen_b,
+                            int e0, int e1, int n_type, int e2, int n_year, int n_month, int n_day, int n_hour, int e3,
+                            float* d_sen_w, float* d_sen_b, float* d_type_tab,
+                            float* d_year_tab, float* d_month_tab, float* d_day_tab, float* d_hour_tab, float* ws, nrm_stream_t stream) {
+    if (nrows0 > 0) if (int rc = check_fe("nrm_frontend_bwd_tables", nrows0, xcols0, P, n_sub, behaviour0, e0, e1, e2, e3)) return rc;
+    if (nrows1 > 0) if (int rc = check_fe("nrm_frontend_bwd_tables", nrows1, xcols1, P, n_sub, behaviour1, e0, e1, e2, e3)) return rc;
+    if (nrows0 < 0 || nrows1 < 0 || (long)nrows0 + nrows1 >= (1L << 31) - 64) return fail(NRM_EINVAL, "nrm_frontend_bwd_tables: nrows=%d,%d", nrows0, nrows1);
+    if ((nrows0 > 0 && (!x0 || !dlab0 || lddl0 < e0 + e1 + e2 + e3)) || (nrows1 > 0 && (!x1 || !dlab1 || lddl1 < e0 + e1 + e2 + e3)))
+        return fail(NRM_EINVAL, "nrm_frontend_bwd_tables: null pointer or lddl too small");
+    if (!sen_w || !sen_b || !d_sen_w || !d_sen_b || !d_type_tab || !d_year_tab || !d_month_tab || !d_day_tab || !d_hour_tab || !ws)
+        return fail(NRM_EINVAL, "nrm_frontend_bwd_tables: null pointer");
+    nrm::FrontendParams p = tab_dims(n_sub, e1, n_type, e2, n_year, n_month, n_day, n_hour, e3);
+    p.e0 = e0; p.P = P; p.n_cat = 1;
+    p.sen_w = sen_w; p.sen_b = sen_b;
+    p.d_sen_w = d_sen_w; p.d_sen_b = d_sen_b; p.d_type_tab = d_type_tab;
+    p.d_year_tab = d_year_tab; p.d_month_tab = d_month_tab; p.d_day_tab = d_day_tab; p.d_hour_tab = d_hour_tab;
+    if (nrm::tab_grad_ws_floats(p, (long)nrows0 + nrows1) <= 0 && nrows0 + nrows1 > 0)
+        return fail(NRM_EINVAL, "nrm_frontend_bwd_tables: shape not taken (nrm_frontend_tables_ws_floats is 0): use nrm_frontend_bwd");
+    return check_hip(nrm::tab_grad_launch(p, x0, nrows0, xcols0, dlab0, lddl0, x1, nrows1, xcols1, dlab1, lddl1, x_is_f64, ws,
+                                          (hipStream_t)stream), "frontend_bwd_tables");
 }
 
 long nrm_frontend_cat_ws_ints(int n_cat, long nrows_total, int n_sub) {
diff --git a/news_recommendation_model_amd/csrc/frontend.hip b/news_recommendation_model_amd/csrc/frontend.hip
--- a/news_recommendation_model_amd/csrc/frontend.hip
+++ b/news_recommendation_model_amd/csrc/frontend.hip
@@ -19,23 +19,23 @@
 };
 
 template <typename XT>
-__device__ __forceinline__ void stage_headers(const FrontendParams& p, const XT* __restrict__ x, int r_lo, int nr, const RowHeaders& hd,
-                                              int nthreads) {
+__device__ __forceinline__ void stage_headers(const FrontendParams& p, int xcols, int* err, const XT* __restrict__ x, int r_lo, int nr,
+                                              const RowHeaders& hd, int nthreads) {
     const int P = p.P, NS = p.n_sub;
     const int c_cat = 4 + P, c_sub = c_cat + 1, c_sen = c_sub + NS, c_typ = c_sen + 3;
     const int items = 9 + NS;
     for (int i = threadIdx.x; i < nr * items; i += nthreads) {
         const int r = i / items, k = i - r * items;
-        const XT* xr = x + (size_t)(r_lo + r) * p.xcols;
+        const XT* xr = x + (size_t)(r_lo + r) * xcols;
         if (k < 4) {
             const int lim = k == 0 ? p.n_year : k == 1 ? p.n_month : k == 2 ? p.n_day : p.n_hour;
-            hd.idx[r * FE_HDR + k] = row_index(xr, k, lim, p.err);
+            hd.idx[r * FE_HDR + k] = row_index(xr, k, lim, err);
         } else if (k == 4) {
-            hd.idx[r * FE_HDR + 4] = row_index(xr, c_cat, p.n_cat, p.err);
+            hd.idx[r * FE_HDR + 4] = row_index(xr, c_cat, p.n_cat, err);
         } else if (k == 5) {
-            hd.idx[r * FE_HDR + 5] = row_index(xr, c_typ, p.n_type, p.err);
+            hd.idx[r * FE_HDR + 5] = row_index(xr, c_typ, p.n_type, err);
         } else if (k < 6 + NS) {
-            hd.idx[r * FE_HDR + k] = row_index(xr, c_sub + (k - 6), p.n_cat, p.err);
+            hd.idx[r * FE_HDR + k] = row_index(xr, c_sub + (k - 6), p.n_cat, err);
         } else {
             hd.sen[r * 4 + (k - 6 - NS)] = (float)xr[c_sen + (k - 6 - NS)];
         }
@@ -51,7 +51,7 @@
     __shared__ float h_sen[FWD_ROWS * 4];
     const int r_lo = blockIdx.x * FWD_ROWS, nr = min(FWD_ROWS, nrows - r_lo);
     const RowHeaders hd = {h_idx, h_sen};
-    stage_headers(p, x, r_lo, nr, hd, FE_THREADS);
+    stage_headers(p, p.xcols, p.err, x, r_lo, nr, hd, FE_THREADS);
     __syncthreads();
     const int P = p.P, NS = p.n_sub;
     const int c_beh = 4 + P + 1 + NS + 3 + 1;
@@ -105,9 +105,7 @@
     const int total = (int)(a_sen + e1 * 4 - sm);
     const RowHeaders hd = {reinterpret_cast<int*>(sm + total), sm + total + FE_ROWS * FE_HDR};
     for (int i = threadIdx.x; i < total; i += FE_THREADS) sm[i] = 0.f;
-    FrontendParams pq = p;
     int dummy = 0;
-    pq.err = &dummy;
     const int NS = p.n_sub;
     const float inv_ns = 1.0f / (float)NS;
     const int small = e1 + e2 + e3;
@@ -115,7 +113,7 @@
     for (int grp = blockIdx.x; grp < ngroups; grp += gridDim.x) {
         const int r_lo = grp * FE_ROWS, nr = min(FE_ROWS, nrows - r_lo);
         __syncthreads();
-        stage_headers(pq, x, r_lo, nr, hd, FE_THREADS);
+        stage_headers(p, p.xcols, &dummy, x, r_lo, nr, hd, FE_THREADS);
         __syncthreads();
         const float* g0 = dlab + (size_t)r_lo * lddl;
         for (int i = threadIdx.x; i < (p.d_cat_tab ? nr * e0 : 0); i += FE_THREADS) {
@@ -126,7 +124,7 @@
             const float gs = gv * inv_ns;
             for (int k = 0; k < NS; ++k) atomicAdd(p.d_cat_tab + (size_t)hi[6 + k] * e0 + c, gs);
         }
-        for (int i = threadIdx.x; i < nr * small; i += FE_THREADS) {
+        for (int i = threadIdx.x; i < (p.d_type_tab ? nr * small : 0); i += FE_THREADS) {
             const int r = i / small, cs = i - r * small;
             const float gv = g0[(size_t)r * lddl + e0 + cs];
             const int* hi = hd.idx + r * FE_HDR;
@@ -151,6 +149,7 @@
         }
     }
     __syncthreads();
+    if (!p.d_type_tab) return;
     for (int i = threadIdx.x; i < p.n_type * e2; i += FE_THREADS) if (a_type[i] != 0.f) atomicAdd(p.d_type_tab + i, a_type[i]);
     for (int i = threadIdx.x; i < p.n_year * e3; i += FE_THREADS) if (a_year[i] != 0.f) atomicAdd(p.d_year_tab + i, a_year[i]);
     for (int i = threadIdx.x; i < p.n_month * e3; i += FE_THREADS) if (a_month[i] != 0.f) atomicAdd(p.d_month_tab + i, a_month[i]);
@@ -192,6 +191,280 @@
         if (shm > 64 * 1024) { hipError_t e = hipFuncSetAttribute((const void*)frontend_bwd_kernel<float>, hipFuncAttributeMaxDynamicSharedMemorySize, (int)shm); if (e != hipSuccess) return e; }
         hipLaunchKernelGGL(frontend_bwd_kernel<float>, grid, dim3(FE_THREADS), shm, st, p, (const float*)x, dlab, lddl, nrows);
     }
+    return hipGetLastError();
+}
+
+constexpr int TB_THREADS = 512;
+constexpr int TB_WAVES = TB_THREADS / 64;
+constexpr int TB_ROWS = 32;
+constexpr int TB_MAXT = 16;
+constexpr int TB_MAXTILES = TB_WAVES * TB_MAXT;
+constexpr int TB_WG_PER_CU = 2;
+constexpr int TB_CB = 4;
+constexpr int TB_RED_CELLS = 64, TB_RED_SLICES = 16;
+
+struct TabTile {
+    short hdr, ibase;
+    short coff, ncol;
+    int dst;
+    short ldr, ldc;
+};
+struct TabSet { const void* x; const float* dlab; int nrows, xcols, lddl, nchunks; };
+struct TabParams {
+    FrontendParams p;
+    TabSet set[2];
+    int ntiles, tiles_per_wave, cells, ldb, chunks_per_wg;
+    float* ws;
+    TabTile tile[TB_MAXTILES];
+};
+
+__device__ __forceinline__ bool fe_finite(float v) { return fabsf(v) <= 3.402823466e+38f; }
+
+template <typename XT, int NT>
+__global__ __launch_bounds__(TB_THREADS, TB_WG_PER_CU * TB_WAVES / 4) void tab_grad_kernel(const TabParams q) {
+    extern __shared__ float sm[];
+    const FrontendParams& p = q.p;
+    const int e0 = p.e0, e1 = p.e1, e2 = p.e2, e3 = p.e3;
+    const int small = e1 + e2 + e3, ldb = q.ldb;
+    float* s_b = sm;
+    float* s_wb = s_b + TB_ROWS * ldb;
+    float* s_sen = s_wb + 4 * e1;
+    float* s_sa = s_sen + TB_ROWS * 4;
+    int* s_idx = reinterpret_cast<int*>(s_sa + TB_ROWS * 4);
+    const RowHeaders hd = {s_idx, s_sen};
+    const int lane = threadIdx.x & 63, wave = __builtin_amdgcn_readfirstlane(threadIdx.x >> 6);
+    const int li = lane & 15, lk = lane >> 4;
+
+    for (int i = threadIdx.x; i < e1 * 4; i += TB_THREADS) s_wb[i] = (i & 3) < 3 ? p.sen_w[(i >> 2) * 3 + (i & 3)] : p.sen_b[i >> 2];
+
+    const int t_lo = wave * q.tiles_per_wave;
+    const int my_nt = max(0, min(q.tiles_per_wave, q.ntiles - t_lo));
+    int t_desc[NT];
+    f32x4 acc[NT];
+#pragma unroll
+    for (int t = 0; t < NT; ++t) {
+        const TabTile& d = q.tile[min(t_lo + t, TB_MAXTILES - 1)];
+        const int v = t < my_nt ? (d.hdr + 1) | (d.ibase << 3) | (d.coff << 18) : 1 | (0x7fff << 3);
+        t_desc[t] = __builtin_amdgcn_readfirstlane(v);
+        acc[t] = f32x4{0.f, 0.f, 0.f, 0.f};
+    }
+
+    int dummy = 0;
+    const int nchunks = q.set[0].nchunks + q.set[1].nchunks;
+    const int ch_lo = blockIdx.x * q.chunks_per_wg, ch_hi = min(nchunks, ch_lo + q.chunks_per_wg);
+    for (int ch = ch_lo; ch < ch_hi; ++ch) {
+        const int si = ch >= q.set[0].nchunks;
+        const TabSet& set = q.set[si];
+        const int r_lo = (ch - (si ? q.set[0].nchunks : 0)) * TB_ROWS, nr = min(TB_ROWS, set.nrows - r_lo);
+        const int nr4 = (nr + 3) & ~3;
+        const float* g0 = set.dlab + (size_t)r_lo * set.lddl + e0;
+        __syncthreads();
+        for (int cb = 0; cb < small; cb += 64 * TB_CB) {
+            float gvs[TB_ROWS / TB_WAVES][TB_CB];
+#pragma unroll
+            for (int k = 0; k < TB_ROWS / TB_WAVES; ++k)
+#pragma unroll
+                for (int u = 0; u < TB_CB; ++u) {
+                    const int r = wave + k * TB_WAVES, c = cb + 64 * u + lane;
+                    gvs[k][u] = (r < nr && c < small) ? g0[(size_t)r * set.lddl + c] : 0.f;
+                }
+            if (cb == 0) {
+                stage_headers(p, set.xcols, &dummy, reinterpret_cast<const XT*>(set.x), r_lo, nr, hd, TB_THREADS);
+                __syncthreads();
+                for (int i = threadIdx.x; i < nr4 * 4; i += TB_THREADS) {
+                    const int r = i >> 2, k = i & 3;
+                    const bool ok = r < nr && fe_finite(s_sen[r * 4]) && fe_finite(s_sen[r * 4 + 1]) && fe_finite(s_sen[r * 4 + 2]);
+                    s_sa[i] = ok ? (k < 3 ? s_sen[i] : 1.f) : 0.f;
+                }
+                for (int i = nr * FE_HDR + threadIdx.x; i < nr4 * FE_HDR; i += TB_THREADS) s_idx[i] = -1;
+            }
+#pragma unroll
+            for (int k = 0; k < TB_ROWS / TB_WAVES; ++k) {
+                const int r = wave + k * TB_WAVES;
+                if (r >= nr4) break;
+                const int* hi = s_idx + r * FE_HDR;
+#pragma unroll
+                for (int u = 0; u < TB_CB; ++u) {
+                    const int c = cb + 64 * u + lane;
+                    if (c >= small) break;
+                    const float gv = gvs[k][u];
+                    float v = 0.f;
+                    if (r < nr) {
+                        const bool fin = fe_finite(gv);
+                        if (c < e1) {
+                            const float s0 = s_sen[r * 4], s1 = s_sen[r * 4 + 1], s2 = s_sen[r * 4 + 2];
+                            const f32x4 wb = *reinterpret_cast<const f32x4*>(s_wb + 4 * c);
+                            const float pre = wb[3] + wb[0] * s0 + wb[1] * s1 + wb[2] * s2;
+                            const bool on = pre > 0.f && gv != 0.f;
+                            const bool slow = !fin || !(fe_finite(s0) && fe_finite(s1) && fe_finite(s2));
+                            if (__ballot(slow)) {
+                                if (slow && on) {
+                                    atomicAdd(p.d_sen_w + c * 3 + 0, gv * s0);
+                                    atomicAdd(p.d_sen_w + c * 3 + 1, gv * s1);
+                                    atomicAdd(p.d_sen_w + c * 3 + 2, gv * s2);
+                                    atomicAdd(p.d_sen_b + c, gv);
+                                }
+                            }
+                            v = (on && !slow) ? gv : 0.f;
+                        } else {
+                            if (__ballot(!fin)) {
+                                if (!fin) {
+                                    if (c < e1 + e2) {
+                                        atomicAdd(p.d_type_tab + hi[5] * e2 + (c - e1), gv);
+                                    } else {
+                                        const int kk = c - e1 - e2;
+                                        atomicAdd(p.d_year_tab + hi[0] * e3 + kk, gv);
+                                        atomicAdd(p.d_month_tab + hi[1] * e3 + kk, gv);
+                                        atomicAdd(p.d_day_tab + hi[2] * e3 + kk, gv);
+                                        atomicAdd(p.d_hour_tab + hi[3] * e3 + kk, gv);
+                                    }
+                                }
+                            }
+                            v = fin ? gv : 0.f;
+                        }
+                    }
+                    s_b[r * ldb + c] = v;
+                }
+            }
+        }
+        __syncthreads();
+        const int* s_a = reinterpret_cast<const int*>(s_sa);
+        const int a_sen = lk * 4 + (li & 3), a_idx = TB_ROWS * 4 + lk * FE_HDR;
+        for (int r0 = 0; r0 < nr4; r0 += 4) {
+            float b[NT];
+            int raw[NT];
+#pragma unroll
+            for (int t = 0; t < NT; ++t) {
+                int d = t_desc[t];
+                asm volatile("" : "+s"(d));
+                const int hdr = (d & 7) - 1, coff = d >> 18;
+                b[t] = s_b[(r0 + lk) * ldb + coff + li];
+                raw[t] = s_a[hdr >= 0 ? r0 * FE_HDR + a_idx + hdr : r0 * 4 + a_sen];
+            }
+#pragma unroll
+            for (int t = 0; t < NT; ++t) {
+                int d = t_desc[t];
+                asm volatile("" : "+s"(d));
+                const int m = (d & 7) ? -1 : 0, ibase = (d >> 3) & 0x7fff;
+                const int one_hot = raw[t] == ibase + li ? __float_as_int(1.f) : 0, sen = li < 4 ? raw[t] : 0;
+                acc[t] = mfma16(__int_as_float((one_hot & m) | (sen & ~m)), b[t], acc[t]);
+            }
+        }
+    }
+    float* part = q.ws + (size_t)blockIdx.x * q.cells;
+#pragma unroll
+    for (int t = 0; t < NT; ++t) {
+        if (t < my_nt) {
+            const TabTile& d = q.tile[t_lo + t];
+            const int nrow = d.hdr >= 0 ? min(16, (d.hdr == 5 ? p.n_type : d.hdr == 0 ? p.n_year : d.hdr == 1 ? p.n_month : d.hdr == 2 ? p.n_day : p.n_hour) - d.ibase) : 4;
+#pragma unroll
+            for (int k = 0; k < 4; ++k) {
+                const int row = 4 * lk + k;
+                if (row < nrow && li < d.ncol) part[d.dst + row * d.ldr + li * d.ldc] = acc[t][k];
+            }
+        }
+    }
+}
+
+__global__ __launch_bounds__(TB_RED_CELLS * TB_RED_SLICES) void tab_reduce_kernel(const FrontendParams p, const float* __restrict__ ws, int nparts, int cells) {
+    __shared__ float s[TB_RED_SLICES][TB_RED_CELLS];
+    const int cl = threadIdx.x & (TB_RED_CELLS - 1), slice = threadIdx.x / TB_RED_CELLS;
+    const int cell = blockIdx.x * TB_RED_CELLS + cl;
+    const int per = (nparts + TB_RED_SLICES - 1) / TB_RED_SLICES;
+    float v = 0.f;
+    if (cell < cells) {
+        const int g_hi = min(nparts, (slice + 1) * per);
+        int g = slice * per;
+        for (; g + 8 <= g_hi; g += 8) {
+            float t[8];
+#pragma unroll
+            for (int k = 0; k < 8; ++k) t[k] = ws[(size_t)(g + k) * cells + cell];
+#pragma unroll
+            for (int k = 0; k < 8; ++k) v += t[k];
+        }
+        for (; g < g_hi; ++g) v += ws[(size_t)g * cells + cell];
+    }
+    s[slice][cl] = v;
+    __syncthreads();
+    if (slice || cell >= cells) return;
+    v = s[0][cl];
+#pragma unroll
+    for (int k = 1; k < TB_RED_SLICES; ++k) v += s[k][cl];
+    int i = cell;
+    float* dst;
+    if (i < p.n_type * p.e2) dst = p.d_type_tab + i;
+    else if ((i -= p.n_type * p.e2) < p.n_year * p.e3) dst = p.d_year_tab + i;
+    else if ((i -= p.n_year * p.e3) < p.n_month * p.e3) dst = p.d_month_tab + i;
+    else if ((i -= p.n_month * p.e3) < p.n_day * p.e3) dst = p.d_day_tab + i;
+    else if ((i -= p.n_day * p.e3) < p.n_hour * p.e3) dst = p.d_hour_tab + i;
+    else { i -= p.n_hour * p.e3; dst = (i & 3) < 3 ? p.d_sen_w + (i >> 2) * 3 + (i & 3) : p.d_sen_b + (i >> 2); }
+    *dst += v;
+}
+
+struct TabPlan { int ntiles, cells, ldb; size_t shm; };
+static bool tab_plan(const FrontendParams& p, TabPlan* pl) {
+    if (p.e1 <= 0 || p.e2 <= 0 || p.e3 <= 0 || p.n_type <= 0 || p.n_year <= 0 || p.n_month <= 0 || p.n_day <= 0 || p.n_hour <= 0) return false;
+    const long n_time = (long)p.n_year + p.n_month + p.n_day + p.n_hour;
+    if (n_time > 30000 || p.n_type > 30000 || (long)p.e1 + p.e2 + p.e3 > 4096) return false;
+    auto up = [](int n) { return (n + 15) / 16; };
+    const long tiles = (long)up(p.e1) + (long)up(p.n_type) * up(p.e2) +
+                       (long)(up(p.n_year) + up(p.n_month) + up(p.n_day) + up(p.n_hour)) * up(p.e3);
+    if (tiles > TB_MAXTILES) return false;
+    const int small = p.e1 + p.e2 + p.e3;
+    pl->ntiles = (int)tiles;
+    pl->cells = p.n_type * p.e2 + (int)n_time * p.e3 + 4 * p.e1;
+    pl->ldb = (small + 63) / 64 * 64 + 16;
+    pl->shm = sizeof(float) * ((size_t)TB_ROWS * pl->ldb + 4 * (size_t)p.e1 + (size_t)TB_ROWS * (8 + FE_HDR));
+    return pl->shm <= 64 * 1024;
+}
+
+static void tab_grid(long nrows0, long nrows1, int* grid, int* chunks_per_wg) {
+    const long nchunks = (nrows0 + TB_ROWS - 1) / TB_ROWS + (nrows1 + TB_ROWS - 1) / TB_ROWS;
+    const long cap = (long)TB_WG_PER_CU * device_cus();
+    const long per = std::max<long>(1, (nchunks + cap - 1) / cap);
+    *chunks_per_wg = (int)per;
+    *grid = (int)((nchunks + per - 1) / per);
+}
+
+long tab_grad_ws_floats(const FrontendParams& p, long nrows_total) {
+    TabPlan pl;
+    if (nrows_total <= 0 || nrows_total >= (1L << 31) - 2 * TB_ROWS || p.n_sub > FE_MAXSUB || !tab_plan(p, &pl)) return 0;
+    const long nchunks = (nrows_total + TB_ROWS - 1) / TB_ROWS + 1;
+    return std::min<long>(nchunks, (long)TB_WG_PER_CU * device_cus()) * pl.cells;
+}
+
+hipError_t tab_grad_launch(const FrontendParams& p, const void* x0, int nrows0, int xcols0, const float* dlab0, int lddl0,
+                           const void* x1, int nrows1, int xcols1, const float* dlab1, int lddl1, int x_is_f64, float* ws, hipStream_t st) {
+    if ((long)nrows0 + nrows1 <= 0) return hipSuccess;
+    TabParams q = {};
+    TabPlan pl;
+    if (p.n_sub > FE_MAXSUB || !tab_plan(p, &pl)) return hipErrorInvalidValue;
+    q.p = p;
+    q.set[0] = {x0, dlab0, nrows0, xcols0, lddl0, (nrows0 + TB_ROWS - 1) / TB_ROWS};
+    q.set[1] = {x1, dlab1, nrows1, xcols1, lddl1, (nrows1 + TB_ROWS - 1) / TB_ROWS};
+    q.ntiles = pl.ntiles; q.cells = pl.cells; q.ldb = pl.ldb; q.ws = ws;
+    q.tiles_per_wave = (pl.ntiles + TB_WAVES - 1) / TB_WAVES;
+    int grid = 0;
+    tab_grid(nrows0, nrows1, &grid, &q.chunks_per_wg);
+    int nt = 0, cell = 0;
+    auto table = [&](int hdr, int n, int e, int coff) {
+        for (int ib = 0; ib < n; ib += 16)
+            for (int c = 0; c < e; c += 16)
+                q.tile[nt++] = {(short)hdr, (short)ib, (short)(coff + c), (short)std::min(16, e - c), cell + ib * e + c, (short)e, 1};
+        cell += n * e;
+    };
+    table(5, p.n_type, p.e2, p.e1);
+    table(0, p.n_year, p.e3, p.e1 + p.e2);
+    table(1, p.n_month, p.e3, p.e1 + p.e2);
+    table(2, p.n_day, p.e3, p.e1 + p.e2);
+    table(3, p.n_hour, p.e3, p.e1 + p.e2);
+    for (int c = 0; c < p.e1; c += 16) q.tile[nt++] = {-1, 0, (short)c, (short)std::min(16, p.e1 - c), cell + 4 * c, 1, 4};
+    if (nt != pl.ntiles || cell + 4 * p.e1 != pl.cells) return hipErrorInvalidValue;
+    auto launch = [&](auto kernel) { hipLaunchKernelGGL(kernel, dim3(grid), dim3(TB_THREADS), pl.shm, st, q); };
+    if (q.tiles_per_wave <= 4)      x_is_f64 ? launch(tab_grad_kernel<double, 4>) : launch(tab_grad_kernel<float, 4>);
+    else if (q.tiles_per_wave <= 8) x_is_f64 ? launch(tab_grad_kernel<double, 8>) : launch(tab_grad_kernel<float, 8>);
+    else                            x_is_f64 ? launch(tab_grad_kernel<double, TB_MAXT>) : launch(tab_grad_kernel<float, TB_MAXT>);
+    hipLaunchKernelGGL(tab_reduce_kernel, dim3((pl.cells + TB_RED_CELLS - 1) / TB_RED_CELLS), dim3(TB_RED_CELLS * TB_RED_SLICES), 0, st, p, ws, grid, pl.cells);
     return hipGetLastError();
 }
 
@@ -300,7 +573,92 @@
     flush(cur);
 }
 
-long cat_grad_ws_ints(int n_cat, long nrows_total, int n_sub) { return 3L * n_cat + 4 + 3L * nrows_total * (n_sub + 1); }
+constexpr int CAT_LDS_MAX = 16384;
+constexpr int CAT_SLICE = 4096;
+constexpr int CAT_MAX_GROUPS = 256;
+static int cat_groups(long nref) { return (int)std::max<long>(1, std::min<long>(CAT_MAX_GROUPS, (nref + CAT_SLICE - 1) / CAT_SLICE)); }
+
+template <typename XT>
+__global__ __launch_bounds__(1024) void cat_hist_kernel(const CatRefs p, int slice, int* __restrict__ hist, int* __restrict__ cat_of) {
+    extern __shared__ int h[];
+    for (int i = threadIdx.x; i < p.n_cat; i += 1024) h[i] = 0;
+    __syncthreads();
+    const int S = p.NS + 1;
+    const long lo_l = (long)blockIdx.x * slice, hi_l = lo_l + slice;
+    const int lo = (int)(lo_l < p.nref ? lo_l : p.nref), hi = (int)(hi_l < p.nref ? hi_l : p.nref);
+    for (int i = lo + threadIdx.x; i < hi; i += 1024) {
+        int r = i / S;
+        const int j = i - r * S;
+        const int set = r >= p.nrows[0];
+        if (set) r -= p.nrows[0];
+        const XT* xr = reinterpret_cast<const XT*>(p.x[set]) + (size_t)r * p.xcols[set];
+        int c = (int)xr[p.c_cat + j];
+        c = c < 0 ? 0 : (c >= p.n_cat ? p.n_cat - 1 : c);
+        cat_of[i] = c;
+        atomicAdd(h + c, 1);
+    }
+    __syncthreads();
+    for (int i = threadIdx.x; i < p.n_cat; i += 1024) hist[(size_t)blockIdx.x * p.n_cat + i] = h[i];
+}
+
+__global__ __launch_bounds__(256) void cat_colscan_kernel(int* __restrict__ hist, int* __restrict__ count, int groups, int n_cat) {
+    __shared__ int part[4][64];
+    const int cl = threadIdx.x & 63, q = threadIdx.x >> 6;
+    const int c = blockIdx.x * 64 + cl;
+    const int per = (groups + 3) / 4, g_lo = min(groups, q * per), g_hi = min(groups, g_lo + per);
+    int sum = 0;
+    if (c < n_cat) {
+        int g = g_lo;
+        for (; g + 8 <= g_hi; g += 8) {
+            int t[8];
+#pragma unroll
+            for (int k = 0; k < 8; ++k) t[k] = hist[(size_t)(g + k) * n_cat + c];
+#pragma unroll
+            for (int k = 0; k < 8; ++k) sum += t[k];
+        }
+        for (; g < g_hi; ++g) sum += hist[(size_t)g * n_cat + c];
+    }
+    part[q][cl] = sum;
+    __syncthreads();
+    if (c >= n_cat) return;
+    int run = 0;
+    for (int k = 0; k < q; ++k) run += part[k][cl];
+    if (q == 3) count[c] = run + sum;
+    int g = g_lo;
+    for (; g + 8 <= g_hi; g += 8) {
+        int t[8];
+#pragma unroll
+        for (int k = 0; k < 8; ++k) t[k] = hist[(size_t)(g + k) * n_cat + c];
+#pragma unroll
+        for (int k = 0; k < 8; ++k) { hist[(size_t)(g + k) * n_cat + c] = run; run += t[k]; }
+    }
+    for (; g < g_hi; ++g) {
+        const int v = hist[(size_t)g * n_cat + c];
+        hist[(size_t)g * n_cat + c] = run;
+        run += v;
+    }
+}
+
+__global__ __launch_bounds__(1024) void cat_place_kernel(long nref, int slice, int n_cat, const int* __restrict__ cat_of,
+                                                         const int* __restrict__ start, const int* __restrict__ hist,
+                                                         int* __restrict__ refs, int* __restrict__ refcat) {
+    extern __shared__ int h[];
+    for (int i = threadIdx.x; i < n_cat; i += 1024) h[i] = start[i] + hist[(size_t)blockIdx.x * n_cat + i];
+    __syncthreads();
+    const long lo_l = (long)blockIdx.x * slice, hi_l = lo_l + slice;
+    const int lo = (int)(lo_l < nref ? lo_l : nref), hi = (int)(hi_l < nref ? hi_l : nref);
+    for (int i = lo + threadIdx.x; i < hi; i += 1024) {
+        const int c = cat_of[i];
+        const int pos = atomicAdd(h + c, 1);
+        refs[pos] = i;
+        refcat[pos] = c;
+    }
+}
+
+long cat_grad_ws_ints(int n_cat, long nrows_total, int n_sub) {
+    const long nref = nrows_total * (n_sub + 1);
+    return 3L * n_cat + 4 + 3L * nref + (n_cat <= CAT_LDS_MAX ? (long)cat_groups(nref) * n_cat : 0);
+}
 
 hipError_t cat_grad_launch(const void* x0, int nrows0, int xcols0, const float* dlab0, int lddl0,
                            const void* x1, int nrows1, int xcols1, const float* dlab1, int lddl1, int x_is_f64,
@@ -318,13 +676,25 @@
     int* cat_of = ws + 3 * n_cat + 4;
     int* refs = cat_of + p.nref;
     int* refcat = refs + p.nref;
-    hipError_t e = hipMemsetAsync(count, 0, sizeof(int) * 2 * (size_t)n_cat, st);
-    if (e != hipSuccess) return e;
-    const unsigned blocks = (unsigned)std::min<long>((p.nref + 255) / 256, 2048);
-    if (x_is_f64) hipLaunchKernelGGL(cat_count_kernel<double>, dim3(blocks), dim3(256), 0, st, p, count, cat_of);
-    else          hipLaunchKernelGGL(cat_count_kernel<float>, dim3(blocks), dim3(256), 0, st, p, count, cat_of);
-    hipLaunchKernelGGL(cat_scan_kernel, dim3(1), dim3(1024), 0, st, count, start, n_cat);
-    hipLaunchKernelGGL(cat_fill_kernel, dim3(blocks), dim3(256), 0, st, p.nref, cat_of, start, cursor, refs, refcat);
+    if (n_cat <= CAT_LDS_MAX) {
+        int* hist = refcat + p.nref;
+        const int groups = cat_groups(p.nref);
+        const int slice = (int)((p.nref + groups - 1) / groups);
+        const size_t shm = sizeof(int) * (size_t)n_cat;
+        if (x_is_f64) hipLaunchKernelGGL(cat_hist_kernel<double>, dim3(groups), dim3(1024), shm, st, p, slice, hist, cat_of);
+        else          hipLaunchKernelGGL(cat_hist_kernel<float>, dim3(groups), dim3(1024), shm, st, p, slice, hist, cat_of);
+        hipLaunchKernelGGL(cat_colscan_kernel, dim3((n_cat + 63) / 64), dim3(256), 0, st, hist, count, groups, n_cat);
+        hipLaunchKernelGGL(cat_scan_kernel, dim3(1), dim3(1024), 0, st, count, start, n_cat);
+        hipLaunchKernelGGL(cat_place_kernel, dim3(groups), dim3(1024), shm, st, p.nref, slice, n_cat, cat_of, start, hist, refs, refcat);
+    } else {
+        hipError_t e = hipMemsetAsync(count, 0, sizeof(int) * 2 * (size_t)n_cat, st);
+        if (e != hipSuccess) return e;
+        const unsigned blocks = (unsigned)std::min<long>((p.nref + 255) / 256, 2048);
+        if (x_is_f64) hipLaunchKernelGGL(cat_count_kernel<double>, dim3(blocks), dim3(256), 0, st, p, count, cat_of);
+        else          hipLaunchKernelGGL(cat_count_kernel<float>, dim3(blocks), dim3(256), 0, st, p, count, cat_of);
+        hipLaunchKernelGGL(cat_scan_kernel, dim3(1), dim3(1024), 0, st, count, start, n_cat);
+        hipLaunchKernelGGL(cat_fill_kernel, dim3(blocks), dim3(256), 0, st, p.nref, cat_of, start, cursor, refs, refcat);
+    }
     const long chunks = (p.nref + 63) / 64;
     hipLaunchKernelGGL(cat_gather_kernel, dim3((unsigned)((chunks + 3) / 4)), dim3(256), 0, st, p, refs, refcat, d_cat);
     return hipGetLastError();
diff --git a/news_recommendation_model_amd/csrc/frontend.hpp b/news_recommendation_model_amd/csrc/frontend.hpp
--- a/news_recommendation_model_amd/csrc/frontend.hpp
+++ b/news_recommendation_model_amd/csrc/frontend.hpp
@@ -15,6 +15,9 @@
 hipError_t frontend_fwd_launch(const FrontendParams& p, const void* x, int x_is_f64, int nrows, hipStream_t st);
 hipError_t frontend_bwd_launch(const FrontendParams& p, const void* x, int x_is_f64, const float* dlab, int lddl,
                                int nrows, hipStream_t st);
+long tab_grad_ws_floats(const FrontendParams& p, long nrows_total);
+hipError_t tab_grad_launch(const FrontendParams& p, const void* x0, int nrows0, int xcols0, const float* dlab0, int lddl0,
+                           const void* x1, int nrows1, int xcols1, const float* dlab1, int lddl1, int x_is_f64, float* ws, hipStream_t st);
 long cat_grad_ws_ints(int n_cat, long nrows_total, int n_sub);
 hipError_t cat_grad_launch(const void* x0, int nrows0, int xcols0, const float* dlab0, int lddl0,
                            const void* x1, int nrows1, int xcols1, const float* dlab1, int lddl1, int x_is_f64,
diff --git a/news_recommendation_model_amd/native.py b/news_recommendation_model_amd/native.py
--- a/news_recommendation_model_amd/native.py
+++ b/news_recommendation_model_amd/native.py
@@ -73,6 +73,9 @@
     "nrm_frontend_fwd": (_c_i, [_c_fp, _c_i, _c_i, _c_i, _c_i, _c_i, _c_i,  _c_fp, _c_i, _c_i,  _c_fp, _c_fp, _c_i,
                                  _c_fp, _c_i, _c_i,  _c_fp, _c_fp, _c_fp, _c_fp,  _c_i, _c_i, _c_i, _c_i, _c_i,
                                  _c_fp, _c_i, _c_fp, _c_i, _c_fp, _c_fp]),
+    "nrm_frontend_tables_ws_floats": (_c_l, [_c_l] + [_c_i] * 9),
+    "nrm_frontend_bwd_tables": (_c_i, [_c_fp, _c_i, _c_i, _c_i, _c_fp, _c_i] * 2 + [_c_i] * 3 + [_c_fp, _c_fp] + [_c_i] * 9
+                                + [_c_fp] * 8 + [_c_fp]),
     "nrm_frontend_cat_ws_ints": (_c_l, [_c_i, _c_l, _c_i]),
     "nrm_frontend_cat_grad": (_c_i, [_c_fp, _c_i, _c_i, _c_fp, _c_i] * 2 + [_c_i] * 5 + [_c_fp, _c_fp, _c_fp]),
     "nrm_frontend_bwd": (_c_i, [_c_fp, _c_i, _c_i, _c_i, _c_i, _c_i, _c_i,  _c_fp, _c_i, _c_fp, _c_fp]
diff --git a/news_recommendation_model_amd/ops.py b/news_recommendation_model_amd/ops.py
--- a/news_recommendation_model_amd/ops.py
+++ b/news_recommendation_model_amd/ops.py
@@ -1617,15 +1617,28 @@
     sort = (forced != "0" and (forced == "1" or refs * e0 >= FE_SORT_MIN_ATOMICS) and 1 <= n_sub <= 16 and e0 <= 512
             and len({x.dtype for _, x, _ in prepared}) == 1 and refs < (1 << 31))
     st = native.stream_ptr()
-    for dlab, x, behaviour in prepared:
+    one_dtype = len({x.dtype for _, x, _ in prepared}) == 1
+    rows = sum(x.shape[0] for _, x, _ in prepared)
+    (dl0, x0, beh0), (dl1, x1, beh1) = prepared[0], (prepared[1] if len(prepared) > 1 else (None, None, False))
+    tab_ws = 0
+    if _os.environ.get("NRM_FE_TABLES") != "0" and one_dtype and len(prepared) <= 2:
+        tab_ws = native.load().nrm_frontend_tables_ws_floats(rows, n_sub, e1, n_type, e2, n_year, n_month, n_day, n_hour, e3)
+    small = (None,) * 7 if tab_ws else tuple(native.ptr(g) for g in (d_sw, d_sb, d_type, d_year, d_month, d_day, d_hour))
+    if tab_ws:
+        ws = torch.empty(tab_ws, dtype=torch.float32, device=dev)
+        native.call("nrm_frontend_bwd_tables", native.ptr(x0), x0.shape[0], x0.shape[1], 1 if beh0 else 0, native.ptr(dl0), dl0.stride(0),
+                    native.ptr(x1) if x1 is not None else None, x1.shape[0] if x1 is not None else 0,
+                    x1.shape[1] if x1 is not None else 0, 1 if beh1 else 0, native.ptr(dl1) if x1 is not None else None,
+                    dl1.stride(0) if x1 is not None else 0, 1 if x0.dtype == torch.float64 else 0, P, n_sub,
+                    native.ptr(sen_w), native.ptr(sen_b), e0, e1, n_type, e2, n_year, n_month, n_day, n_hour, e3,
+                    native.ptr(d_sw), native.ptr(d_sb), native.ptr(d_type), native.ptr(d_year), native.ptr(d_month),
+                    native.ptr(d_day), native.ptr(d_hour), native.ptr(ws), st)
+    for dlab, x, behaviour in (prepared if not (tab_ws and sort) else ()):
         native.call("nrm_frontend_bwd", native.ptr(x), 1 if x.dtype == torch.float64 else 0, x.shape[0], x.shape[1], P,
                     n_sub, 1 if behaviour else 0, native.ptr(dlab), dlab.stride(0), native.ptr(sen_w), native.ptr(sen_b),
                     n_cat, e0, e1, n_type, e2, n_year, n_month, n_day, n_hour, e3,
-                    None if sort else native.ptr(d_cat), native.ptr(d_sw), native.ptr(d_sb), native.ptr(d_type),
-                    native.ptr(d_year), native.ptr(d_month), native.ptr(d_day), native.ptr(d_hour), st)
+                    None if sort else native.ptr(d_cat), *small, st)
     if sort:
-        (dl0, x0, _), (dl1, x1, _) = prepared[0], (prepared[1] if len(prepared) > 1 else (None, None, None))
-        rows = x0.shape[0] + (x1.shape[0] if x1 is not None else 0)
         ws = torch.empty(native.load().nrm_frontend_cat_ws_ints(n_cat, rows, n_sub), dtype=torch.int32, device=dev)
         native.call("nrm_frontend_cat_grad", native.ptr(x0), x0.shape[0], x0.shape[1], native.ptr(dl0), dl0.stride(0),
                     native.ptr(x1) if x1 is not None else None, x1.shape[0] if x1 is not None else 0,
```

Result: faster. 35800, median of 6 (+1.3%).
